# xmlyqing00/V-FloodNet

Hardware: AMD Instinct MI355X
Metric: segmented frames/sec at 480p (higher is better)
Workload: dtype f32

## Files before the change

v-floodnet_amd/_lib.py:

```python
import ctypes as C
import os
import re

import torch

_HERE = os.path.dirname(os.path.abspath(__file__))
LIB_PATH = os.environ.get('VFN_LIB_PATH') or os.path.join(_HERE, 'libvfn_hip.so')

_lib = None

c_fp = C.c_void_p

_SCALARS = {'int': C.c_int, 'float': C.c_float, 'double': C.c_double, 'long long': C.c_longlong}
_POINTEES = set(_SCALARS) | {'void', 'char', 'unsigned char', 'short', 'unsigned short', 'unsigned long long'}
_RENAMED = {'in': 'inp'}
_DECLARATOR = re.compile(r'(?:const\s+)?([A-Za-z_][\w ]*?)(?:\s*(\*)\s*|\s+)(\w+)\s*(?:\[([^\]]*)\])?')


def parse_header(text):
    defines, enums, structs, protos = {}, {}, {}, {}

    def fail(why, decl):
        raise RuntimeError(f'vfn_hip.h: {why}: {" ".join(decl.split())[:120]!r}')

    def number(expr, decl):
        try:
            if not re.fullmatch(r'[\w\s()+*-]+', expr):
                raise ValueError(expr)
            return int(eval(expr, {'__builtins__': {}}, {**defines, **enums}))
        except Exception:
            fail(f'cannot evaluate {expr.strip()!r}', decl)

    def declarator(item, decl, param):
        m = _DECLARATOR.fullmatch(item.strip())
        if not m:
            fail('declaration not understood', decl)
        base, star, name, bound = ' '.join(m.group(1).split()), m.group(2), m.group(3), m.group(4)
        if base not in _POINTEES and base not in structs:
            fail(f'unknown base type {base!r}', decl)
        if bound is not None and (star or param):
            fail('array of pointers or array parameter', decl)
        if star:
            if base == 'char':
                t = C.c_char_p
            elif base in structs and param and not name.endswith('_dev'):
                t = C.POINTER(structs[base])
            else:
                t = C.c_void_p
        elif base in _SCALARS:
            t = _SCALARS[base]
        elif base in structs and not param:
            t = structs[base]
        else:
            fail(f'{base!r} by value', decl)
        return _RENAMED.get(name, name), t if bound is None else t * number(bound, decl)

    text = re.sub(r'/\*.*?\*/', ' ', text, flags=re.S)
    text = re.sub(r'//[^\n]*', ' ', text)
    text = re.sub(r'^[ \t]*#[ \t]*ifdef[ \t]+__cplusplus\b.*?^[ \t]*#[ \t]*endif\b[^\n]*$', ' ', text, flags=re.S | re.M)
    code = []
    for line in text.split('\n'):
        if not line.lstrip().startswith('#'):
            code.append(line)
        elif not re.fullmatch(r'\s*#\s*(ifndef\s+\w+|define\s+\w+|endif)\s*', line):
            m = re.fullmatch(r'\s*#\s*define\s+(\w+)\b(?!\()(.+)', line)
            if not m:
                fail('directive not understood', line)
            defines[m.group(1)] = number(m.group(2), line)
    text = '\n'.join(code)

    decls, depth, start = [], 0, 0
    for pos, ch in enumerate(text):
        depth += (ch == '{') - (ch == '}')
        if depth < 0:
            fail('unbalanced declaration', text[start:pos + 1])
        if ch == ';' and depth == 0:
            decls.append(text[start:pos])
            start = pos + 1
    if text[start:].strip():
        fail('unbalanced declaration', text[start:])

    for decl in decls:
        m = re.fullmatch(r'\s*enum\s*\{(.*)\}\s*', decl, flags=re.S)
        if m:
            value = -1
            for item in m.group(1).split(','):
                name, _, expr = item.partition('=')
                value = number(expr, decl) if expr.strip() else value + 1
                enums[name.strip()] = value
            continue
        m = re.fullmatch(r'\s*typedef\s+struct\s*(\w*)\s*\{(.*)\}\s*(\w+)\s*', decl, flags=re.S)
        if m:
            if m.group(1) not in ('', m.group(3)):
                fail('struct tag and typedef name differ', decl)
            fields = []
            for member in m.group(2).split(';'):
                if member.strip():
                    first, *more = member.split(',')
                    head = _DECLARATOR.fullmatch(first.strip())
                    if more and (not head or head.group(2)):
                        fail('several declarators after a pointer', member)
                    fields.append(declarator(first, member, False))
                    fields += [declarator(f'{head.group(1)} {item}', member, False) for item in more]
            structs[m.group(3)] = type(m.group(3), (C.Structure,), {'_fields_': fields})
            continue
        m = re.fullmatch(r'\s*int\s+(vfn_\w+)\s*\((.*)\)\s*', decl, flags=re.S)
        if m:
            if m.group(1) in protos:
                fail('declared twice', decl)
            params = m.group(2).strip()
            protos[m.group(1)] = [] if params == 'void' else [declarator(p, decl, True)[1] for p in params.split(',')]
            continue
        fail('declaration not understood', decl)
    return defines, enums, structs, protos


with open(os.path.join(os.path.dirname(_HERE), 'include', 'vfn_hip.h')) as _f:
    DEFINES, ENUMS, STRUCTS, SIGNATURES = parse_header(_f.read())
ALL_SYMBOLS = sorted(SIGNATURES)
with open(os.path.join(os.path.dirname(_HERE), 'include', 'vfn_winograd6.h')) as _f:
    SIGNATURES_WINOGRAD6 = parse_header(_f.read())[3]
with open(os.path.join(os.path.dirname(_HERE), 'include', 'vfn_image_val.h')) as _f:
    DEFINES_IMAGE_VAL, _, _, SIGNATURES_IMAGE_VAL = parse_header(_f.read())
SEG_SCORES_CHUNK, SEG_SCORES_MAX_BLOCKS = DEFINES_IMAGE_VAL['VFN_SEG_SCORES_CHUNK'], DEFINES_IMAGE_VAL['VFN_SEG_SCORES_MAX_BLOCKS']
ABI_VERSION = DEFINES['VFN_ABI_VERSION']
TRAIN_AUG_MAX_T, TRAIN_AUG_MAX_SIDE, TRAIN_AUG_MAX_OUT, TRAIN_AUG_MAX_OBJ = (
    DEFINES['VFN_TRAIN_AUG_MAX_' + _k] for _k in ('T', 'SIDE', 'OUT', 'OBJ'))

ConvDesc = STRUCTS['vfn_conv_desc']
WgradDesc = STRUCTS['vfn_wgrad_desc']
RefreshFilter = STRUCTS['vfn_refresh_filter']
RefreshEpilogue = STRUCTS['vfn_refresh_epilogue']
GatherEntry = STRUCTS['vfn_gather_entry']
StemDesc = STRUCTS['vfn_stem_desc']
BankScanDesc = STRUCTS['vfn_bankscan_desc']
MemReadDesc = STRUCTS['vfn_memread_desc']
BankMatchDesc = STRUCTS['vfn_bankmatch_desc']
BankDesc = STRUCTS['vfn_bank_desc']
TrainAugFrame = STRUCTS['vfn_train_aug_frame']
TrainAugDesc = STRUCTS['vfn_train_aug_desc']

DESC_IDS = {ENUMS['VFN_DESC_' + _k]: _c for _k, _c in (
    ('CONV', ConvDesc), ('STEM', StemDesc), ('BANKSCAN', BankScanDesc), ('MEMREAD', MemReadDesc), ('BANK', BankDesc),
    ('WGRAD', WgradDesc), ('REFRESH_FILTER', RefreshFilter), ('REFRESH_EPILOGUE', RefreshEpilogue), ('GATHER', GatherEntry),
    ('BANKMATCH', BankMatchDesc), ('TRAIN_AUG', TrainAugDesc))}


def lib():
    global _lib
    if _lib is None:
        if not os.path.isfile(LIB_PATH):
            raise RuntimeError(
                f'{LIB_PATH} not found: build the HIP kernels first '
                '(python -c "import __graft_entry__ as g; g.build()" or make -C v-floodnet_amd/csrc)')
        L = C.CDLL(LIB_PATH)

        def declare(name, signatures=SIGNATURES, header='vfn_hip.h'):
            if not hasattr(L, name):
                raise RuntimeError(f'{LIB_PATH} lacks {name}, which include/{header} declares: rebuild it (make -C v-floodnet_amd/csrc)')
            fn = getattr(L, name)
            fn.argtypes, fn.restype = signatures[name], C.c_int
            return fn

        if declare('vfn_abi_version')() != ABI_VERSION:
            raise RuntimeError(f'{LIB_PATH} has ABI version {L.vfn_abi_version()}, this package expects {ABI_VERSION} '
                               '(descriptor layouts differ): rebuild it (make -C v-floodnet_amd/csrc)')
        declare('vfn_sizeof_desc')
        for which, cls in DESC_IDS.items():
            if L.vfn_sizeof_desc(which) != C.sizeof(cls):
                raise RuntimeError(f'{LIB_PATH}: sizeof({cls.__name__}) is {L.vfn_sizeof_desc(which)} in the library, '
                                   f'{C.sizeof(cls)} in this binding: rebuild it (make -C v-floodnet_amd/csrc)')
        for name in SIGNATURES:
            declare(name)
        for name in SIGNATURES_WINOGRAD6:
            declare(name, SIGNATURES_WINOGRAD6, 'vfn_winograd6.h')
        for name in SIGNATURES_IMAGE_VAL:
            declare(name, SIGNATURES_IMAGE_VAL, 'vfn_image_val.h')
        _lib = L
    return _lib


def check(status, what):
    if status != 0:
        raise RuntimeError(f'HIP kernel launcher {what} failed with status {status}')


def ptr(t):
    if t is None:
        return None
    return C.c_void_p(t.data_ptr())


_raw_stream = getattr(torch._C, '_cuda_getCurrentRawStream', None)


def stream():
    if _raw_stream is not None:
        return C.c_void_p(_raw_stream(torch.cuda.current_device()))
    return C.c_void_p(torch.cuda.current_stream().cuda_stream)


def require_gpu(t, what='tensor'):
    if not t.is_cuda:
        raise RuntimeError(f'{what} must live on the GPU: the V-FloodNet hot path has no CPU fallback')


PROBES = []


def independent_stream(device, beside=(), tries=12, priority=0):
    device = torch.device(device)
    cur = torch.cuda.current_stream(device)
    others = [cur] + [s_ for s_ in beside if s_ is not None]
    big, small = torch.zeros(16 * 1024 * 1024, device=device), torch.zeros(16, device=device)

    def overlaps(cand, ref):
        torch.cuda.synchronize(device)
        ref_end, cand_end = torch.cuda.Event(), torch.cuda.Event()
        with torch.cuda.stream(ref):
            for _ in range(64):
                big.add_(1.0)
            ref_end.record()
        with torch.cuda.stream(cand):
            small.add_(1.0)
            cand_end.record()
        cand_end.synchronize()
        ok = not ref_end.query()
        torch.cuda.synchronize(device)
        return ok

    cand = None
    for n_ in range(tries):
        cand = torch.cuda.Stream(device=device, priority=priority)
        if all(overlaps(cand, o_) for o_ in others):
            PROBES.append((True, n_ + 1))
            return cand
    PROBES.append((False, tries))
    import warnings
    warnings.warn('vfloodnet_amd: no stream with a hardware queue of its own found; side-stream work will run in order with the frame loop')
    return cand
```

v-floodnet_amd/csrc/conv_winograd.hip:

```cpp
#include "common.h"
#include "conv_internal.h"
#include "../../include/vfn_hip.h"
#include "../../include/vfn_winograd6.h"

namespace {

__device__ __forceinline__ void bt6(const f32x4 (&v)[6], f32x4 (&t)[6]) {
    t[0] = 4.f * v[0] - 5.f * v[2] + v[4];
    t[1] = -4.f * (v[1] + v[2]) + v[3] + v[4];
    t[2] = 4.f * (v[1] - v[2]) - v[3] + v[4];
    t[3] = -2.f * v[1] - v[2] + 2.f * v[3] + v[4];
    t[4] = 2.f * v[1] - v[2] - 2.f * v[3] + v[4];
    t[5] = 4.f * v[1] - 5.f * v[3] + v[5];
}

template <bool LPOUT = false>
__global__ __launch_bounds__(256)
void winograd_input_kernel(const float* __restrict__ x, int N, int H, int W, int C, int ld_x, int relu, float* __restrict__ V,
                           int rows_pad) {
    const int th = (H + 3) / 4, tw = (W + 3) / 4;
    const int c4n = C / 4;
    const long long total = (long long)N * th * tw * c4n;
    const __amdgpu_buffer_rsrc_t rx = __builtin_amdgcn_make_buffer_rsrc(const_cast<float*>(x), 0, (int)((size_t)N * H * W * ld_x * 4), 0x00020000);
    const float floor_ = relu ? 0.f : -INFINITY;
    for (long long i = vfn_xcd_block(blockIdx.x, gridDim.x) * (long long)blockDim.x + threadIdx.x; i < total; i += (long long)gridDim.x * blockDim.x) {
        const int c4 = (int)(i % c4n);
        const int tile = (int)(i / c4n);
        const int tx = tile % tw, ty = (tile / tw) % th, n = tile / (tw * th);
        f32x4 d[6][6];
#pragma unroll
        for (int a = 0; a < 6; ++a) {
            const int yy = 4 * ty - 1 + a;
#pragma unroll
            for (int b = 0; b < 6; ++b) {
                const int xx = 4 * tx - 1 + b;
                const bool ok = (unsigned)yy < (unsigned)H && (unsigned)xx < (unsigned)W;
                const int off = ok ? (((n * H + yy) * W + xx) * ld_x + c4 * 4) * 4 : 0x7ffffff0;
                d[a][b] = __builtin_bit_cast(f32x4, __builtin_amdgcn_raw_buffer_load_b128(rx, off, 0, 0));
            }
        }
#pragma unroll
        for (int a = 0; a < 6; ++a)
#pragma unroll
            for (int b = 0; b < 6; ++b)
#pragma unroll
                for (int e = 0; e < 4; ++e) d[a][b][e] = vfn_floor_nan(d[a][b][e], floor_);
#pragma unroll
        for (int b = 0; b < 6; ++b) {
            f32x4 v[6], t[6];
#pragma unroll
            for (int a = 0; a < 6; ++a) v[a] = d[a][b];
            bt6(v, t);
#pragma unroll
            for (int a = 0; a < 6; ++a) d[a][b] = t[a];
        }
#pragma unroll
        for (int a = 0; a < 6; ++a) {
            f32x4 t[6];
            bt6(d[a], t);
#pragma unroll
            for (int b = 0; b < 6; ++b) {
                if constexpr (LPOUT) {
                    const vfn_bf16x4 h = {(__bf16)t[b][0], (__bf16)t[b][1], (__bf16)t[b][2], (__bf16)t[b][3]};
                    *reinterpret_cast<vfn_bf16x4*>(reinterpret_cast<__bf16*>(V) + ((size_t)(a * 6 + b) * rows_pad + tile) * C + c4 * 4) = h;
                } else {
                    *reinterpret_cast<f32x4*>(V + ((size_t)(a * 6 + b) * rows_pad + tile) * C + c4 * 4) = t[b];
                }
            }
        }
    }
}

__device__ __forceinline__ void at6(const f32x4 (&m)[6], f32x4 (&y)[4]) {
    const f32x4 s12 = m[1] + m[2], d12 = m[1] - m[2], s34 = m[3] + m[4], d34 = m[3] - m[4];
    y[0] = m[0] + s12 + s34;
    y[1] = d12 + 2.f * d34;
    y[2] = s12 + 4.f * s34;
    y[3] = d12 + 8.f * d34 + m[5];
}

template <bool MASK>
__global__ __launch_bounds__(256)
void winograd_output_kernel(const float* __restrict__ Mb, int rows_pad, int N, int H, int W, int Cout,
                            const float* __restrict__ scale, const float* __restrict__ shift, const float* __restrict__ res, int res_ld,
                            int res_mod, int relu_out, float* __restrict__ out, int out_ld, const float* __restrict__ mask, int mask_ld,
                            int mask_after) {
    const int th = (H + 3) / 4, tw = (W + 3) / 4;
    const int c4n = Cout / 4;
    const long long total = (long long)N * th * tw * c4n;
    const int npix = N * H * W;
    const __amdgpu_buffer_rsrc_t ro = __builtin_amdgcn_make_buffer_rsrc(out, 0, (int)((size_t)npix * out_ld * 4), 0x00020000);
    const __amdgpu_buffer_rsrc_t rr = __builtin_amdgcn_make_buffer_rsrc(const_cast<float*>(res ? res : Mb), 0,
                                                                        res ? (int)((size_t)(res_mod > 0 ? res_mod : npix) * res_ld * 4) : 0, 0x00020000);
    const __amdgpu_buffer_rsrc_t rm = __builtin_amdgcn_make_buffer_rsrc(const_cast<float*>(MASK ? mask : Mb), 0,
                                                                        MASK ? (int)((size_t)npix * mask_ld * 4) : 0, 0x00020000);
    const float floor_ = relu_out ? 0.f : -INFINITY;
    for (long long i = vfn_xcd_block(blockIdx.x, gridDim.x) * (long long)blockDim.x + threadIdx.x; i < total; i += (long long)gridDim.x * blockDim.x) {
        const int c4 = (int)(i % c4n);
        const int tile = (int)(i / c4n);
        const int tx = tile % tw, ty = (tile / tw) % th, n = tile / (tw * th);
        f32x4 m[6][6];
#pragma unroll
        for (int a = 0; a < 6; ++a)
#pragma unroll
            for (int b = 0; b < 6; ++b) m[a][b] = *reinterpret_cast<const f32x4*>(Mb + ((size_t)(a * 6 + b) * rows_pad + tile) * Cout + c4 * 4);
        f32x4 sc = {1.f, 1.f, 1.f, 1.f}, sh = {0.f, 0.f, 0.f, 0.f};
        if (scale) sc = *reinterpret_cast<const f32x4*>(scale + c4 * 4);
        if (shift) sh = *reinterpret_cast<const f32x4*>(shift + c4 * 4);
        f32x4 t[6][4];
#pragma unroll
        for (int a = 0; a < 6; ++a) at6(m[a], t[a]);
        int rowi[4][4];
#pragma unroll
        for (int a = 0; a < 4; ++a)
#pragma unroll
            for (int b = 0; b < 4; ++b) {
                const int yy = 4 * ty + a, xx = 4 * tx + b;
                rowi[a][b] = (yy < H && xx < W) ? (n * H + yy) * W + xx : -1;
            }
        f32x4 rv[4][4], mk[MASK ? 4 : 1][MASK ? 4 : 1];
#pragma unroll
        for (int a = 0; a < 4; ++a)
#pragma unroll
            for (int b = 0; b < 4; ++b) {
                const int row = rowi[a][b];
                const int rrow = res_mod > 0 ? row % res_mod : row;
                rv[a][b] = __builtin_bit_cast(f32x4, __builtin_amdgcn_raw_buffer_load_b128(rr, row >= 0 ? (rrow * res_ld + c4 * 4) * 4 : 0x7ffffff0, 0, 0));
                if constexpr (MASK)
                    mk[a][b] = __builtin_bit_cast(f32x4, __builtin_amdgcn_raw_buffer_load_b128(rm, row >= 0 ? (row * mask_ld + c4 * 4) * 4 : 0x7ffffff0, 0, 0));
            }
#pragma unroll
        for (int b = 0; b < 4; ++b) {
            f32x4 col[6], y[4];
#pragma unroll
            for (int a = 0; a < 6; ++a) col[a] = t[a][b];
            at6(col, y);
#pragma unroll
            for (int a = 0; a < 4; ++a) {
                f32x4 v;
#pragma unroll
                for (int e = 0; e < 4; ++e) v[e] = y[a][e] * sc[e] + sh[e];
                if constexpr (MASK) {
                    if (!mask_after) {
#pragma unroll
                        for (int e = 0; e < 4; ++e) v[e] = mk[a][b][e] > 0.f ? v[e] : 0.f;
                    }
                }
                v += rv[a][b];
                if constexpr (MASK) {
                    if (mask_after) {
#pragma unroll
                        for (int e = 0; e < 4; ++e) v[e] = mk[a][b][e] > 0.f ? v[e] : 0.f;
                    }
                }
#pragma unroll
                for (int e = 0; e < 4; ++e) v[e] = vfn_floor_nan(v[e], floor_);
                const int row = rowi[a][b];
                __builtin_amdgcn_raw_buffer_store_b128(__builtin_bit_cast(__attribute__((ext_vector_type(4))) unsigned, v), ro,
                                                       row >= 0 ? (row * out_ld + c4 * 4) * 4 : 0x7ffffff0, 0, 0);
            }
        }
    }
}

typedef float f32x2 __attribute__((ext_vector_type(2)));
typedef unsigned u32x2 __attribute__((ext_vector_type(2)));

__device__ __forceinline__ void bt8(const f32x2 (&v)[8], f32x2 (&t)[8]) {
    const f32x2 e1 = v[2] + v[6] - 4.25f * v[4], o1 = v[1] + v[5] - 4.25f * v[3];
    const f32x2 e2 = v[6] + 0.25f * v[2] - 1.25f * v[4], o2 = 0.5f * v[1] - 2.5f * v[3] + 2.f * v[5];
    const f32x2 e3 = v[6] + 4.f * v[2] - 5.f * v[4], o3 = 2.f * v[1] - 2.5f * v[3] + 0.5f * v[5];
    t[0] = v[0] - v[6] + 5.25f * (v[4] - v[2]);
    t[1] = e1 + o1;
    t[2] = e1 - o1;
    t[3] = e2 + o2;
    t[4] = e2 - o2;
    t[5] = e3 + o3;
    t[6] = e3 - o3;
    t[7] = v[7] - v[1] + 5.25f * (v[3] - v[5]);
}

inline int winograd6_tiles(int N, int H, int W) { return N * ((H + 5) / 6) * ((W + 5) / 6); }

__global__ __launch_bounds__(256, 2)
void winograd6_input_kernel(const float* __restrict__ x, int N, int H, int W, int C, int ld_x, int relu, float* __restrict__ V,
                            int rows_pad) {
    const int th = (H + 5) / 6, tw = (W + 5) / 6, tiles = N * th * tw;
    const int c2n = C / 2;
    const long long total = (long long)rows_pad * c2n;
    const __amdgpu_buffer_rsrc_t rx = __builtin_amdgcn_make_buffer_rsrc(const_cast<float*>(x), 0, (int)((size_t)N * H * W * ld_x * 4), 0x00020000);
    const __amdgpu_buffer_rsrc_t rv = __builtin_amdgcn_make_buffer_rsrc(V, 0, (int)((size_t)64 * rows_pad * C * 4), 0x00020000);
    const int comp4 = rows_pad * C * 4;
    const float floor_ = relu ? 0.f : -INFINITY;
    const long long i = vfn_xcd_block(blockIdx.x, gridDim.x) * (long long)blockDim.x + threadIdx.x;
    if (i >= total) return;
    {
        const int c2 = (int)(i % c2n);
        const int tile = (int)(i / c2n);
        const int vo = (tile * C + c2 * 2) * 4;
        if (tile >= tiles) {
#pragma unroll
            for (int xi = 0; xi < 64; ++xi) __builtin_amdgcn_raw_buffer_store_b64(u32x2{0u, 0u}, rv, vo, xi * comp4, 0);
            return;
        }
        const int tx = tile % tw, ty = (tile / tw) % th, n = tile / (tw * th);
        const int y0 = 6 * ty - 1, x0 = 6 * tx - 1;
        const int base = (((n * H + y0) * W + x0) * ld_x + c2 * 2) * 4;
        f32x2 d[8][8];
#pragma unroll
        for (int a = 0; a < 8; ++a) {
#pragma unroll
            for (int b = 0; b < 8; ++b) {
                const bool ok = (unsigned)(y0 + a) < (unsigned)H && (unsigned)(x0 + b) < (unsigned)W;
                d[a][b] = __builtin_bit_cast(f32x2, __builtin_amdgcn_raw_buffer_load_b64(rx, ok ? base + (a * W + b) * ld_x * 4 : 0x7ffffff0, 0, 0));
            }
        }
#pragma unroll
        for (int a = 0; a < 8; ++a)
#pragma unroll
            for (int b = 0; b < 8; ++b)
#pragma unroll
                for (int e = 0; e < 2; ++e) d[a][b][e] = vfn_floor_nan(d[a][b][e], floor_);
#pragma unroll
        for (int b = 0; b < 8; ++b) {
            f32x2 v[8], t[8];
#pragma unroll
            for (int a = 0; a < 8; ++a) v[a] = d[a][b];
            bt8(v, t);
#pragma unroll
            for (int a = 0; a < 8; ++a) d[a][b] = t[a];
        }
#pragma unroll
        for (int a = 0; a < 8; ++a) {
            f32x2 t[8];
            bt8(d[a], t);
#pragma unroll
            for (int b = 0; b < 8; ++b) __builtin_amdgcn_raw_buffer_store_b64(__builtin_bit_cast(u32x2, t[b]), rv, vo, (a * 8 + b) * comp4, 0);
        }
    }
}

__device__ __forceinline__ void at8(const f32x2 (&m)[8], f32x2 (&y)[6]) {
    const f32x2 s12 = m[1] + m[2], d12 = m[1] - m[2], s34 = m[3] + m[4], d34 = m[3] - m[4], s56 = m[5] + m[6], d56 = m[5] - m[6];
    y[0] = m[0] + s12 + s34 + s56;
    y[1] = d12 + 2.f * d34 + 0.5f * d56;
    y[2] = s12 + 4.f * s34 + 0.25f * s56;
    y[3] = d12 + 8.f * d34 + 0.125f * d56;
    y[4] = s12 + 16.f * s34 + 0.0625f * s56;
    y[5] = d12 + 32.f * d34 + 0.03125f * d56 + m[7];
}

template <bool RES>
__global__ __launch_bounds__(256, RES ? 1 : 2)
void winograd6_output_kernel(const float* __restrict__ Mb, int rows_pad, int N, int H, int W, int Cout,
                             const float* __restrict__ scale, const float* __restrict__ shift, const float* __restrict__ res, int res_ld,
                             int res_mod, int relu_out, float* __restrict__ out, int out_ld) {
    const int th = (H + 5) / 6, tw = (W + 5) / 6;
    const int c2n = Cout / 2;
    const long long total = (long long)N * th * tw * c2n;
    const int npix = N * H * W;
    const __amdgpu_buffer_rsrc_t rm = __builtin_amdgcn_make_buffer_rsrc(const_cast<float*>(Mb), 0, (int)((size_t)64 * rows_pad * Cout * 4), 0x00020000);
    const __amdgpu_buffer_rsrc_t ro = __builtin_amdgcn_make_buffer_rsrc(out, 0, (int)((size_t)npix * out_ld * 4), 0x00020000);
    const __amdgpu_buffer_rsrc_t rr = __builtin_amdgcn_make_buffer_rsrc(const_cast<float*>(res ? res : Mb), 0,
                                                                        res ? (int)((size_t)(res_mod > 0 ? res_mod : npix) * res_ld * 4) : 0, 0x00020000);
    const float floor_ = relu_out ? 0.f : -INFINITY;
    const int comp4 = rows_pad * Cout * 4;
    const long long i = vfn_xcd_block(blockIdx.x, gridDim.x) * (long long)blockDim.x + threadIdx.x;
    if (i >= total) return;
    {
        int iw = (int)i;
        const int mo = ((iw / c2n) * Cout + (iw % c2n) * 2) * 4;
        f32x2 m[8][8];
#pragma unroll
        for (int a = 0; a < 8; ++a)
#pragma unroll
            for (int b = 0; b < 8; ++b) m[a][b] = __builtin_bit_cast(f32x2, __builtin_amdgcn_raw_buffer_load_b64(rm, mo, (a * 8 + b) * comp4, 0));
        f32x2 t[8][6];
#pragma unroll
        for (int a = 0; a < 8; ++a) at8(m[a], t[a]);
        __builtin_amdgcn_sched_barrier(0);
        asm volatile("" : "+v"(iw));
        const int c2 = iw % c2n, tile = iw / c2n;
        const int tx = tile % tw, ty = (tile / tw) % th, n = tile / (tw * th);
        f32x2 sc = {1.f, 1.f}, sh = {0.f, 0.f};
        if (scale) sc = *reinterpret_cast<const f32x2*>(scale + c2 * 2);
        if (shift) sh = *reinterpret_cast<const f32x2*>(shift + c2 * 2);
        const int y0 = 6 * ty, x0 = 6 * tx, row0 = (n * H + y0) * W + x0;
        const int rb = ((row0 - (res_mod > 0 ? (n * H * W) / res_mod * res_mod : 0)) * res_ld + c2 * 2) * 4;
        f32x2 rv[RES ? 6 : 1][RES ? 6 : 1];
        if constexpr (RES) {
#pragma unroll
            for (int a = 0; a < 6; ++a)
#pragma unroll
                for (int b = 0; b < 6; ++b) {
                    const bool ok = y0 + a < H && x0 + b < W;
                    rv[a][b] = __builtin_bit_cast(f32x2, __builtin_amdgcn_raw_buffer_load_b64(rr, ok ? rb + (a * W + b) * res_ld * 4 : 0x7ffffff0, 0, 0));
                }
        }
        const int oo = (row0 * out_ld + c2 * 2) * 4;
#pragma unroll
        for (int b = 0; b < 6; ++b) {
            f32x2 col[8], y[6];
#pragma unroll
            for (int a = 0; a < 8; ++a) col[a] = t[a][b];
            at8(col, y);
#pragma unroll
            for (int a = 0; a < 6; ++a) {
                f32x2 v;
#pragma unroll
                for (int e = 0; e < 2; ++e) v[e] = vfn_floor_nan(y[a][e] * sc[e] + sh[e] + (RES ? rv[a][b][e] : 0.f), floor_);
                const bool ok = y0 + a < H && x0 + b < W;
                __builtin_amdgcn_raw_buffer_store_b64(__builtin_bit_cast(u32x2, v), ro, ok ? oo + (a * W + b) * out_ld * 4 : 0x7ffffff0, 0, 0);
            }
        }
    }
}

__device__ __forceinline__ void a6(const f32x4 (&v)[4], f32x4 (&z)[6]) {
    const f32x4 e = v[0] + v[2], o = v[1] + v[3];
    const f32x4 e4 = v[0] + 4.f * v[2], o8 = 2.f * v[1] + 8.f * v[3];
    z[0] = v[0];
    z[1] = e + o;
    z[2] = e - o;
    z[3] = e4 + o8;
    z[4] = e4 - o8;
    z[5] = v[3];
}

__global__ __launch_bounds__(256)
void winograd_gy_kernel(const float* __restrict__ gy, int N, int H, int W, int C, int ld, float* __restrict__ Z, int rows_pad) {
    const int th = (H + 3) / 4, tw = (W + 3) / 4;
    const int c4n = C / 4;
    const long long total = (long long)N * th * tw * c4n;
    for (long long i = vfn_xcd_block(blockIdx.x, gridDim.x) * (long long)blockDim.x + threadIdx.x; i < total; i += (long long)gridDim.x * blockDim.x) {
        const int c4 = (int)(i % c4n);
        const int tile = (int)(i / c4n);
        const int tx = tile % tw, ty = (tile / tw) % th, n = tile / (tw * th);
        f32x4 t[6][4];
#pragma unroll
        for (int b = 0; b < 4; ++b) {
            f32x4 col[4], z[6];
            const int xx = 4 * tx + b;
#pragma unroll
            for (int a = 0; a < 4; ++a) {
                const int yy = 4 * ty + a;
                f32x4 v = {0.f, 0.f, 0.f, 0.f};
                if (yy < H && xx < W) v = *reinterpret_cast<const f32x4*>(gy + ((size_t)(n * H + yy) * W + xx) * ld + c4 * 4);
                col[a] = v;
            }
            a6(col, z);
#pragma unroll
            for (int a = 0; a < 6; ++a) t[a][b] = z[a];
        }
#pragma unroll
        for (int a = 0; a < 6; ++a) {
            f32x4 z[6];
            a6(t[a], z);
#pragma unroll
            for (int b = 0; b < 6; ++b)
                *reinterpret_cast<f32x4*>(Z + ((size_t)(a * 6 + b) * rows_pad + tile) * C + c4 * 4) = z[b];
        }
    }
}

__device__ __forceinline__ void gt3(const f32x4 (&u)[6], f32x4 (&w)[3]) {
    const f32x4 s12 = u[1] + u[2], d12 = u[2] - u[1], s34 = u[3] + u[4], d34 = u[3] - u[4];
    w[0] = 0.25f * u[0] - (1.f / 6.f) * s12 + (1.f / 24.f) * s34;
    w[1] = (1.f / 6.f) * d12 + (1.f / 12.f) * d34;
    w[2] = -(1.f / 6.f) * s12 + (1.f / 6.f) * s34 + u[5];
}

__global__ __launch_bounds__(256)
void winograd_dw_kernel(const float* __restrict__ dU, int Cout, int Cin, const float* __restrict__ rowscale, float* __restrict__ dw,
                        int accumulate) {
    const int c4n = Cin / 4;
    const long long total = (long long)Cout * c4n;
    const size_t bank = (size_t)Cout * Cin;
    for (long long i = vfn_xcd_block(blockIdx.x, gridDim.x) * (long long)blockDim.x + threadIdx.x; i < total; i += (long long)gridDim.x * blockDim.x) {
        const int c4 = (int)(i % c4n), co = (int)(i / c4n);
        f32x4 t[3][6];
#pragma unroll
        for (int j = 0; j < 6; ++j) {
            f32x4 u[6], w[3];
#pragma unroll
            for (int a = 0; a < 6; ++a) u[a] = *reinterpret_cast<const f32x4*>(dU + (size_t)(a * 6 + j) * bank + (size_t)co * Cin + c4 * 4);
            gt3(u, w);
#pragma unroll
            for (int a = 0; a < 3; ++a) t[a][j] = w[a];
        }
        const float sc = rowscale ? rowscale[co] : 1.f;
#pragma unroll
        for (int a = 0; a < 3; ++a) {
            f32x4 w[3];
            gt3(t[a], w);
#pragma unroll
            for (int b = 0; b < 3; ++b) {
                f32x4* o = reinterpret_cast<f32x4*>(dw + ((size_t)co * 9 + a * 3 + b) * Cin + c4 * 4);
                f32x4 v = w[b] * sc;
                if (accumulate) v += *o;
                *o = v;
            }
        }
    }
}


struct wino_gemm_args {
    const float* V;
    const float* U;
    float* Mb;
    int comps, rows_pad, C, Cout, cout_pad;
    int mtiles, ntiles;
    int a_ld, out_ld, res_ld, res_mod, relu_in, relu_out;
    const float* scale;
    const float* shift;
    const float* res;
};

template <int BM, int BN, int WM, int WN, int PD, bool CONV = false, bool LP = false>
__global__ __launch_bounds__(WM * WN * 64)
void wino_gemm_kernel(const wino_gemm_args p) {
    static_assert(!(CONV && LP), "the reduced-precision form is the transform-domain GEMM only");
    constexpr int BK = 32;
    constexpr int KT = LP ? 64 : 32;
    constexpr int ES = LP ? 2 : 4;
    constexpr int NT = WM * WN * 64;
    constexpr int TM = BM / WM / 32, TN = BN / WN / 32;
    constexpr int AC = BM * 8 / NT, BC = BN * 8 / NT, RSTEP = NT / 8;
    static_assert(AC >= 1 && BC >= 1, "tile too small for the thread count");
    extern __shared__ __attribute__((aligned(16))) char smem[];
    float* sA = reinterpret_cast<float*>(smem);
    float* sB = sA + 2 * BM * BK;

    const int tid = threadIdx.x, lane = tid & 63, wave = tid >> 6;
    const int wm = wave / WN, wn = wave % WN;
    const int li = lane & 31, lh = lane >> 5;

    const int per = p.mtiles * p.ntiles, total = p.comps * per;
    const int gx = (int)gridDim.x >> 3, xcd = (int)blockIdx.x & 7, loc = (int)blockIdx.x >> 3;
    const int q = total >> 3, r8 = total & 7;
    const int u_begin = xcd < r8 ? xcd * (q + 1) : r8 * (q + 1) + (xcd - r8) * q;
    const int u_end = u_begin + q + (xcd < r8 ? 1 : 0);
    const int first = u_begin + loc;
    const int n_units = first < u_end ? (u_end - first + gx - 1) / gx : 0;
    const int nk = p.C / KT;
    const int T = n_units * nk;
    if (T == 0) return;

    const int c16 = tid & 7, r0 = tid >> 3;
    const int a_ld = CONV ? p.a_ld : p.C;
    const __amdgpu_buffer_rsrc_t rsV = __builtin_amdgcn_make_buffer_rsrc(const_cast<float*>(p.V), 0, (int)((size_t)p.comps * p.rows_pad * a_ld * ES), 0x00020000);
    const __amdgpu_buffer_rsrc_t rsU = __builtin_amdgcn_make_buffer_rsrc(const_cast<float*>(p.U), 0, (int)((size_t)p.comps * p.cout_pad * p.C * ES), 0x00020000);
    int a_thr[AC], b_thr[BC];
#pragma unroll
    for (int j = 0; j < AC; ++j) a_thr[j] = (r0 + j * RSTEP) * a_ld * ES + c16 * 16;
#pragma unroll
    for (int j = 0; j < BC; ++j) b_thr[j] = (r0 + j * RSTEP) * p.C * ES + c16 * 16;

    int lu = 0, lkt = 0, la_base = 0, lb_base = 0;
    int n0_cur = 0;
    auto unit_bases = [&](int ui, int& a_base, int& b_base, size_t& o_base, int* n0 = nullptr) {
        const int u = first + ui * gx;
        const int xi = u / per, rem = u - xi * per;
        const int mt = rem / p.ntiles, nt = rem - mt * p.ntiles;
        a_base = (xi * p.rows_pad + mt * BM) * a_ld * ES;
        b_base = (xi * p.cout_pad + nt * BN) * p.C * ES;
        o_base = CONV ? (size_t)mt * BM : ((size_t)xi * p.rows_pad + mt * BM) * p.Cout + nt * BN;
        if (n0) *n0 = nt * BN;
    };
    size_t o_dummy;
    unit_bases(0, la_base, lb_base, o_dummy);
    f32x4 ra[PD][AC], rb[PD][BC];
    auto request = [&](int slot) {
        const int koff = lkt * 128;
#pragma unroll
        for (int j = 0; j < AC; ++j)
            ra[slot][j] = __builtin_bit_cast(f32x4, __builtin_amdgcn_raw_buffer_load_b128(rsV, a_thr[j], la_base + koff, 0));
#pragma unroll
        for (int j = 0; j < BC; ++j)
            rb[slot][j] = __builtin_bit_cast(f32x4, __builtin_amdgcn_raw_buffer_load_b128(rsU, b_thr[j], lb_base + koff, 0));
        if (++lkt == nk) {
            lkt = 0;
            if (++lu < n_units) unit_bases(lu, la_base, lb_base, o_dummy);
        }
    };
    const float relu_floor = (CONV && p.relu_in) ? 0.f : -INFINITY;
    auto stage = [&](int buf, int slot) {
        float* dA = sA + buf * BM * BK;
        float* dB = sB + buf * BN * BK;
#pragma unroll
        for (int j = 0; j < AC; ++j) {
            const int r = r0 + j * RSTEP;
            f32x4 v = ra[slot][j];
            if constexpr (CONV) {
#pragma unroll
                for (int e = 0; e < 4; ++e) v[e] = fmaxf(v[e], relu_floor);
            }
            *reinterpret_cast<f32x4*>(dA + r * BK + ((c16 ^ ((r >> 1) & 7)) << 2)) = v;
        }
#pragma unroll
        for (int j = 0; j < BC; ++j) {
            const int r = r0 + j * RSTEP;
            *reinterpret_cast<f32x4*>(dB + r * BK + ((c16 ^ ((r >> 1) & 7)) << 2)) = rb[slot][j];
        }
    };

    f32x16 acc[TM][TN];
#pragma unroll
    for (int i = 0; i < TM; ++i)
#pragma unroll
        for (int j = 0; j < TN; ++j)
#pragma unroll
            for (int r = 0; r < 16; ++r) acc[i][j][r] = 0.f;

    int cu = 0, ckt = 0, ca_dummy, cb_dummy;
    size_t o_base;
    unit_bases(0, ca_dummy, cb_dummy, o_base, &n0_cur);

#pragma unroll
    for (int d = 0; d < PD; ++d)
        if (d < T) request(d);
    stage(0, 0);
    __syncthreads();

    for (int t0 = 0; t0 < T; t0 += PD) {
#pragma unroll
        for (int uu = 0; uu < PD; ++uu) {
            const int t = t0 + uu;
            if (t >= T) break;
            const int buf = t & 1;
            const bool more = t + 1 < T;
            const bool more_req = t + PD < T;
            const float* cA = sA + buf * BM * BK + (wm * TM * 32) * BK;
            const float* cB = sB + buf * BN * BK + (wn * TN * 32) * BK;
            auto read_frags = [&](int kk, f32x4 (&a)[TM], f32x4 (&b)[TN]) {
                const int lc = 2 * kk + lh;
#pragma unroll
                for (int i = 0; i < TM; ++i) {
                    const int r = i * 32 + li;
                    a[i] = *reinterpret_cast<const f32x4*>(cA + r * BK + ((lc ^ ((r >> 1) & 7)) << 2));
                }
#pragma unroll
                for (int j = 0; j < TN; ++j) {
                    const int r = j * 32 + li;
                    b[j] = *reinterpret_cast<const f32x4*>(cB + r * BK + ((lc ^ ((r >> 1) & 7)) << 2));
                }
            };
            f32x4 fa[2][TM], fb[2][TN];
            read_frags(0, fa[0], fb[0]);
#pragma unroll
            for (int kk = 0; kk < 4; ++kk) {
                if (PD > 1 && kk == 0 && more) stage(buf ^ 1, (uu + 1) % PD);
                if (kk == 1 && more_req) request(uu);
                if (PD == 1 && kk == 3 && more) stage(buf ^ 1, 0);
                if (kk + 1 < 4) read_frags(kk + 1, fa[(kk + 1) & 1], fb[(kk + 1) & 1]);
                if constexpr (LP) {
                    typedef __attribute__((ext_vector_type(8))) __bf16 bf16x8_;
#pragma unroll
                    for (int i = 0; i < TM; ++i)
#pragma unroll
                        for (int j = 0; j < TN; ++j)
                            acc[i][j] = __builtin_amdgcn_mfma_f32_32x32x16_bf16(__builtin_bit_cast(bf16x8_, fa[kk & 1][i]), __builtin_bit_cast(bf16x8_, fb[kk & 1][j]),
                                                                                acc[i][j], 0, 0, 0);
                } else {
#pragma unroll
                for (int e = 0; e < 4; ++e)
#pragma unroll
                    for (int i = 0; i < TM; ++i)
#pragma unroll
                        for (int j = 0; j < TN; ++j)
                            acc[i][j] = __builtin_amdgcn_mfma_f32_32x32x2f32(fa[kk & 1][i][e], fb[kk & 1][j][e], acc[i][j], 0, 0, 0);
                }
            }
            if (++ckt == nk) {
                if constexpr (CONV) {
                    const int m0 = (int)o_base;
                    const int npix = p.rows_pad;
                    const __amdgpu_buffer_rsrc_t rso = __builtin_amdgcn_make_buffer_rsrc(p.Mb, 0, (int)((size_t)npix * p.out_ld * 4), 0x00020000);
                    const __amdgpu_buffer_rsrc_t rsr = __builtin_amdgcn_make_buffer_rsrc(const_cast<float*>(p.res ? p.res : p.V), 0,
                        p.res ? (int)((size_t)(p.res_mod > 0 ? p.res_mod : npix) * p.res_ld * 4) : 0, 0x00020000);
                    const float floor_ = p.relu_out ? 0.f : -INFINITY;
                    float rv[TM][TN][16];
#pragma unroll
                    for (int j = 0; j < TN; ++j) {
                        const int col = n0_cur + (wn * TN + j) * 32 + li;
#pragma unroll
                        for (int i = 0; i < TM; ++i)
#pragma unroll
                            for (int r = 0; r < 16; ++r) {
                                const int row = m0 + (wm * TM + i) * 32 + 4 * lh + (r & 3) + 8 * (r >> 2);
                                const int rrow = p.res_mod > 0 ? row % p.res_mod : row;
                                rv[i][j][r] = __builtin_bit_cast(float, __builtin_amdgcn_raw_buffer_load_b32(
                                    rsr, (row < npix && col < p.Cout) ? (rrow * p.res_ld + col) * 4 : 0x7ffffff0, 0, 0));
                            }
                    }
#pragma unroll
                    for (int j = 0; j < TN; ++j) {
                        const int col = n0_cur + (wn * TN + j) * 32 + li;
                        const bool cok = col < p.Cout;
                        const float sc = (p.scale && cok) ? p.scale[col] : 1.f;
                        const float sh = (p.shift && cok) ? p.shift[col] : 0.f;
#pragma unroll
                        for (int i = 0; i < TM; ++i)
#pragma unroll
                            for (int r = 0; r < 16; ++r) {
                                const int row = m0 + (wm * TM + i) * 32 + 4 * lh + (r & 3) + 8 * (r >> 2);
                                const float v = vfn_floor_nan(acc[i][j][r] * sc + sh + rv[i][j][r], floor_);
                                __builtin_amdgcn_raw_buffer_store_b32(__builtin_bit_cast(unsigned, v), rso,
                                                                      (row < npix && cok) ? (row * p.out_ld + col) * 4 : 0x7ffffff0, 0, 0);
                                acc[i][j][r] = 0.f;
                            }
                    }
                } else {
                float* o = p.Mb + o_base;
#pragma unroll
                for (int j = 0; j < TN; ++j) {
                    const int col = (wn * TN + j) * 32 + li;
#pragma unroll
                    for (int i = 0; i < TM; ++i) {
                        const int rbase = (wm * TM + i) * 32 + 4 * lh;
#pragma unroll
                        for (int r = 0; r < 16; ++r) {
                            if (n0_cur + col < p.Cout)
                                o[(size_t)(rbase + (r & 3) + 8 * (r >> 2)) * p.Cout + col] = acc[i][j][r];
                            acc[i][j][r] = 0.f;
                        }
                    }
                }
                }
                ckt = 0;
                if (++cu < n_units) unit_bases(cu, ca_dummy, cb_dummy, o_base, &n0_cur);
            }
            __syncthreads();
        }
    }
}

template <int BM, int BN, int WM, int WN, int PD, bool CONV, bool LP>
int launch_wino_gemm(const wino_gemm_args& a, int wgs, hipStream_t s) {
    constexpr size_t lds = 2 * (size_t)(BM + BN) * 32 * sizeof(float);
    static const bool lds_ready = vfn_allow_lds(&wino_gemm_kernel<BM, BN, WM, WN, PD, CONV, LP>, lds);
    (void)lds_ready;
    wino_gemm_args p = a;
    p.mtiles = (a.rows_pad + BM - 1) / BM;
    p.ntiles = (a.Cout + BN - 1) / BN;
    const int total = p.comps * p.mtiles * p.ntiles;
    int grid = wgs > 0 ? wgs : 512;
    if (grid > total) grid = total;
    grid = (grid + 7) / 8 * 8;
    hipLaunchKernelGGL((wino_gemm_kernel<BM, BN, WM, WN, PD, CONV, LP>), dim3(grid), dim3(WM * WN * 64), lds, s, p);
    return vfn_check_launch();
}

constexpr int kWinoTile[4][4] = {{128, 128, 4, 2}, {64, 128, 2, 4}, {128, 64, 4, 2}, {64, 64, 2, 2}};
constexpr int kWinoCfgs = 8;

template <bool CONV, bool LP>
int launch_wino_cfg(const wino_gemm_args& a, int cfg, int wgs, hipStream_t s) {
    return vfn_dispatch<kWinoCfgs>(cfg, [&](auto id) -> int {
        constexpr int c = decltype(id)::value;
        constexpr const int* t = kWinoTile[c & 3];
        return launch_wino_gemm<t[0], t[1], t[2], t[3], 1 + (c >> 2), CONV, LP>(a, wgs, s);
    });
}

inline bool tensors_fit_32bit(int N, int H, int W, int ld, int res_ld, int mask_ld, int res_mod) {
    const long long px = (long long)N * H * W;
    return px * ld * 4 < 0x7fffff00LL && (res_mod > 0 ? (long long)res_mod : px) * res_ld * 4 < 0x7fffff00LL && px * mask_ld * 4 < 0x7fffff00LL;
}

inline int grid_of(long long total) {
    long long b = (total + 255) / 256;
    return (int)(b < 16384 ? (b ? b : 1) : 16384);
}

}

extern "C" int vfn_winograd_tiles(int N, int H, int W) { return N * ((H + 3) / 4) * ((W + 3) / 4); }

extern "C" int vfn_winograd_input_f32(const float* x, int N, int H, int W, int C, int ld_x, int relu, float* V, int rows_pad, void* stream) {
    if (!x || !V || N < 1 || H < 1 || W < 1 || C < 4 || C % 4 || ld_x < C || ld_x % 4 || rows_pad < vfn_winograd_tiles(N, H, W)) return VFN_ERR_ARG;
    const long long total = (long long)vfn_winograd_tiles(N, H, W) * (C / 4);
    if (!tensors_fit_32bit(N, H, W, ld_x, 0, 0, 0)) return VFN_ERR_ARG;
    hipLaunchKernelGGL(winograd_input_kernel<false>, dim3(grid_of(total)), dim3(256), 0, (hipStream_t)stream, x, N, H, W, C, ld_x, relu, V, rows_pad);
    return vfn_check_launch();
}

extern "C" int vfn_winograd_output_f32(const float* Mb, int rows_pad, int N, int H, int W, int Cout, const float* scale, const float* shift,
                                       const float* res, int res_ld, int res_mod, int relu_out, float* out, int out_ld, void* stream) {
    if (!Mb || !out || N < 1 || H < 1 || W < 1 || Cout < 4 || Cout % 4 || out_ld < Cout || out_ld % 4 || (res && res_ld % 4) ||
        rows_pad < vfn_winograd_tiles(N, H, W)) return VFN_ERR_ARG;
    const long long total = (long long)vfn_winograd_tiles(N, H, W) * (Cout / 4);
    if (!tensors_fit_32bit(N, H, W, out_ld, res ? res_ld : 0, 0, res_mod)) return VFN_ERR_ARG;
    hipLaunchKernelGGL(winograd_output_kernel<false>, dim3(grid_of(total)), dim3(256), 0, (hipStream_t)stream, Mb, rows_pad, N, H, W, Cout, scale, shift,
                       res, res_ld, res_mod, relu_out, out, out_ld, (const float*)nullptr, 0, 0);
    return vfn_check_launch();
}

extern "C" int vfn_winograd6_input_f32(const float* x, int N, int H, int W, int C, int ld_x, int relu, float* V, int rows_pad, void* stream) {
    if (!x || !V || N < 1 || H < 1 || W < 1 || C < 4 || C % 4 || ld_x < C || ld_x % 4 || rows_pad < winograd6_tiles(N, H, W)) return VFN_ERR_ARG;
    if (!tensors_fit_32bit(N, H, W, ld_x, 0, 0, 0) || (long long)64 * rows_pad * C * 4 >= 0x7fffff00LL) return VFN_ERR_ARG;
    hipLaunchKernelGGL(winograd6_input_kernel, dim3(((long long)rows_pad * (C / 2) + 255) / 256), dim3(256), 0, (hipStream_t)stream, x, N, H, W, C, ld_x, relu,
                       V, rows_pad);
    return vfn_check_launch();
}

extern "C" int vfn_winograd6_output_f32(const float* Mb, int rows_pad, int N, int H, int W, int Cout, const float* scale, const float* shift,
                                        const float* res, int res_ld, int res_mod, int relu_out, float* out, int out_ld, void* stream) {
    if (!Mb || !out || N < 1 || H < 1 || W < 1 || Cout < 4 || Cout % 4 || out_ld < Cout || out_ld % 4 || (res && res_ld % 4) ||
        rows_pad < winograd6_tiles(N, H, W) || res_mod < 0 || (res && res_mod % (H * W))) return VFN_ERR_ARG;
    if (!tensors_fit_32bit(N, H, W, out_ld, res ? res_ld : 0, 0, res_mod) || (long long)64 * rows_pad * Cout * 4 >= 0x7fffff00LL) return VFN_ERR_ARG;
    const dim3 grid(((long long)winograd6_tiles(N, H, W) * (Cout / 2) + 255) / 256);
    if (res)
        hipLaunchKernelGGL(winograd6_output_kernel<true>, grid, dim3(256), 0, (hipStream_t)stream, Mb, rows_pad, N, H, W, Cout, scale, shift, res, res_ld,
                           res_mod, relu_out, out, out_ld);
    else
        hipLaunchKernelGGL(winograd6_output_kernel<false>, grid, dim3(256), 0, (hipStream_t)stream, Mb, rows_pad, N, H, W, Cout, scale, shift, res, res_ld,
                           res_mod, relu_out, out, out_ld);
    return vfn_check_launch();
}

extern "C" int vfn_winograd_output_masked_f32(const float* Mb, int rows_pad, int N, int H, int W, int Cout, const float* res, int res_ld,
                                              const float* mask, int mask_ld, int mask_after, float* out, int out_ld, void* stream) {
    if (!Mb || !out || N < 1 || H < 1 || W < 1 || Cout < 4 || Cout % 4 || out_ld < Cout || out_ld % 4 || (res && res_ld % 4) ||
        (mask && mask_ld % 4) || rows_pad < vfn_winograd_tiles(N, H, W)) return VFN_ERR_ARG;
    const long long total = (long long)vfn_winograd_tiles(N, H, W) * (Cout / 4);
    if (!tensors_fit_32bit(N, H, W, out_ld, res ? res_ld : 0, mask ? mask_ld : 0, 0)) return VFN_ERR_ARG;
    if (mask)
        hipLaunchKernelGGL(winograd_output_kernel<true>, dim3(grid_of(total)), dim3(256), 0, (hipStream_t)stream, Mb, rows_pad, N, H, W, Cout,
                           (const float*)nullptr, (const float*)nullptr, res, res_ld, 0, 0, out, out_ld, mask, mask_ld, mask_after);
    else
        hipLaunchKernelGGL(winograd_output_kernel<false>, dim3(grid_of(total)), dim3(256), 0, (hipStream_t)stream, Mb, rows_pad, N, H, W, Cout,
                           (const float*)nullptr, (const float*)nullptr, res, res_ld, 0, 0, out, out_ld, (const float*)nullptr, 0, 0);
    return vfn_check_launch();
}

extern "C" int vfn_winograd_gy_f32(const float* gy, int N, int H, int W, int C, int ld, float* Z, int rows_pad, void* stream) {
    if (!gy || !Z || N < 1 || H < 1 || W < 1 || C < 4 || C % 4 || ld < C || ld % 4 || rows_pad < vfn_winograd_tiles(N, H, W)) return VFN_ERR_ARG;
    const long long total = (long long)vfn_winograd_tiles(N, H, W) * (C / 4);
    hipLaunchKernelGGL(winograd_gy_kernel, dim3(grid_of(total)), dim3(256), 0, (hipStream_t)stream, gy, N, H, W, C, ld, Z, rows_pad);
    return vfn_check_launch();
}

extern "C" int vfn_winograd_dw_f32(const float* dU, int Cout, int Cin, const float* rowscale, float* dw, int accumulate, void* stream) {
    if (!dU || !dw || Cout < 1 || Cin < 4 || Cin % 4) return VFN_ERR_ARG;
    hipLaunchKernelGGL(winograd_dw_kernel, dim3(grid_of((long long)Cout * (Cin / 4))), dim3(256), 0, (hipStream_t)stream, dU, Cout, Cin, rowscale,
                       dw, accumulate);
    return vfn_check_launch();
}

extern "C" int vfn_winograd_gemm_f32(const float* V, const float* U, float* Mb, int comps, int rows_pad, int C, int Cout, int cout_pad, int cfg,
                                     int wgs, void* stream) {
    if (!V || !U || !Mb || comps < 1 || rows_pad < 1 || C < 32 || C % 32 || Cout < 1 || cout_pad < Cout || cfg < 0 || cfg >= kWinoCfgs) return VFN_ERR_ARG;
    const int bm = kWinoTile[cfg & 3][0], bn = kWinoTile[cfg & 3][1];
    if (rows_pad % bm || cout_pad < (Cout + bn - 1) / bn * bn) return VFN_ERR_ARG;
    if ((long long)comps * rows_pad * C * 4 >= 0x7fffff00LL || (long long)comps * cout_pad * C * 4 >= 0x7fffff00LL) return VFN_ERR_ARG;
    wino_gemm_args a{V, U, Mb, comps, rows_pad, C, Cout, cout_pad, 0, 0, 0, 0, 0, 0, 0, 0, nullptr, nullptr, nullptr};
    return launch_wino_cfg<false, false>(a, cfg, wgs, (hipStream_t)stream);
}

extern "C" int vfn_conv1x1_persistent_f32(const vfn_conv_desc* d, int cfg, int wgs, void* stream) {
    if (!d || !d->in || !d->w || !d->out || cfg < 0 || cfg >= kWinoCfgs) return VFN_ERR_ARG;
    if (d->KH != 1 || d->KW != 1 || d->stride != 1 || d->pad != 0 || d->mask || d->in_lp || d->out_lp || d->w_packed || d->ksplit > 1 ||
        d->w_batch_rows || d->Cin % 32 || d->in_ld % 4 || d->M < 1 || d->M != d->N * d->H * d->W) return VFN_ERR_ARG;
    const int bn = kWinoTile[cfg & 3][1];
    if (d->cout_pad < (d->Cout + bn - 1) / bn * bn) return VFN_ERR_ARG;
    const long long lim = 0x7fffff00LL;
    if ((long long)d->M * d->in_ld * 4 >= lim || (long long)d->M * d->out_ld * 4 >= lim || (long long)d->cout_pad * d->Cin * 4 >= lim ||
        (d->res && (long long)(d->res_mod > 0 ? d->res_mod : d->M) * d->res_ld * 4 >= lim)) return VFN_ERR_ARG;
    wino_gemm_args a{d->in, d->w, d->out, 1, d->M, d->Cin, d->Cout, d->cout_pad, 0, 0,
                     d->in_ld, d->out_ld, d->res ? d->res_ld : 0, d->res_mod, d->relu_in, d->relu_out, d->scale, d->shift, d->res};
    return launch_wino_cfg<true, false>(a, cfg, wgs, (hipStream_t)stream);
}

extern "C" int vfn_winograd_input_bf16(const float* x, int N, int H, int W, int C, int ld_x, int relu, void* V, int rows_pad, void* stream) {
    if (!x || !V || N < 1 || H < 1 || W < 1 || C < 4 || C % 4 || ld_x < C || ld_x % 4 || rows_pad < vfn_winograd_tiles(N, H, W)) return VFN_ERR_ARG;
    const long long total = (long long)vfn_winograd_tiles(N, H, W) * (C / 4);
    if (!tensors_fit_32bit(N, H, W, ld_x, 0, 0, 0)) return VFN_ERR_ARG;
    hipLaunchKernelGGL(winograd_input_kernel<true>, dim3(grid_of(total)), dim3(256), 0, (hipStream_t)stream, x, N, H, W, C, ld_x, relu,
                       reinterpret_cast<float*>(V), rows_pad);
    return vfn_check_launch();
}

extern "C" int vfn_winograd_gemm_bf16(const void* V, const void* U, float* Mb, int comps, int rows_pad, int C, int Cout, int cout_pad, int cfg,
                                      int wgs, void* stream) {
    if (!V || !U || !Mb || comps < 1 || rows_pad < 1 || C < 64 || C % 64 || Cout < 1 || cout_pad < Cout || cfg < 0 || cfg >= kWinoCfgs) return VFN_ERR_ARG;
    const int bm = kWinoTile[cfg & 3][0], bn = kWinoTile[cfg & 3][1];
    if (rows_pad % bm || cout_pad < (Cout + bn - 1) / bn * bn) return VFN_ERR_ARG;
    if ((long long)comps * rows_pad * C * 2 >= 0x7fffff00LL || (long long)comps * cout_pad * C * 2 >= 0x7fffff00LL) return VFN_ERR_ARG;
    wino_gemm_args a{reinterpret_cast<const float*>(V), reinterpret_cast<const float*>(U), Mb, comps, rows_pad, C, Cout, cout_pad, 0, 0, 0, 0, 0, 0, 0, 0,
                     nullptr, nullptr, nullptr};
    return launch_wino_cfg<false, true>(a, cfg, wgs, (hipStream_t)stream);
}
```

v-floodnet_amd/engine.py:

```python
import math
import os

import torch

from . import _lib, ops, weights as W
from ._lib import ptr, stream, check, MemReadDesc, BankScanDesc
from .feature_bank import pick_nsplit, pick_scan_slices, MAX_SPLIT, MAX_SPLIT_SCAN, QT_SCAN, DK, DV

_CFG_EFF = {(128, 128): 1.00, (128, 64): 0.95, (64, 128): 0.95, (64, 64): 0.86, (32, 64): 0.74,
            (64, 32): 0.74, (128, 32): 0.80, (256, 128): 0.97}
_CFG_TILES = None
_TUNED = {}
_TUNED_PATH = __import__('os').path.join(__import__('os').path.dirname(__import__('os').path.abspath(__file__)),
                                         'tuned_gfx950.json')
_TUNED_BF16 = {}
_TUNED_BF16_PATH = _TUNED_PATH.replace('tuned_gfx950.json', 'tuned_gfx950_bf16.json')
_TUNED_BF16X3 = {}
_TUNED_BF16X3_PATH = _TUNED_PATH.replace('tuned_gfx950.json', 'tuned_gfx950_bf16x3.json')
_TABLES = (_TUNED, _TUNED_BF16, _TUNED_BF16X3)
_TABLE_PATHS = (_TUNED_PATH, _TUNED_BF16_PATH, _TUNED_BF16X3_PATH)
_TUNED_WINO6 = {}
_TUNED_WINO6_PATH = _TUNED_PATH.replace('tuned_gfx950.json', 'tuned_gfx950_wino6.json')


def is_wino6_desc(d):
    return d.w_batch_rows > 0 and d.M == 64 * d.w_batch_rows


def table_of(d, mode):
    return _TUNED_WINO6 if mode == 0 and is_wino6_desc(d) else _TABLES[mode]


def _load_tuned():
    import json
    import os
    if os.environ.get('VFN_IGNORE_TUNED') == '1':
        return
    for path, table in zip(_TABLE_PATHS + (_TUNED_WINO6_PATH,), _TABLES + (_TUNED_WINO6,)):
        alt = os.environ.get('VFN_TUNED_DIR')
        if alt and os.path.isfile(os.path.join(alt, os.path.basename(path))):
            path = os.path.join(alt, os.path.basename(path))
        if os.path.isfile(path):
            for k, v in json.load(open(path)).items():
                t = (int(v[0]), int(v[1]), int(v[2]) if len(v) > 2 else 0)
                table[tuple(int(x) for x in k.split(','))] = t + tuple(int(x) for x in v[3:6]) if len(v) >= 6 else t


def save_tuned(path=None, mode=0):
    import json
    table = _TUNED_WINO6 if mode == 'wino6' else _TABLES[mode]
    with open(path or (_TUNED_WINO6_PATH if mode == 'wino6' else _TABLE_PATHS[mode]), 'w') as f:
        json.dump({','.join(str(x) for x in k): list(v) for k, v in sorted(table.items())}, f, indent=0)


_load_tuned()


def pad_divide_by(h, w, d=16):
    new_h = h + d - h % d if h % d > 0 else h
    new_w = w + d - w % d if w % d > 0 else w
    lh = int((new_h - h) / 2)
    uh = int(new_h - h) - lh
    lw = int((new_w - w) / 2)
    uw = int(new_w - w) - lw
    return (lw, uw, lh, uh), new_h, new_w


WS_FLOATS = 16 * 1024 * 1024
_WINOGRAD_TRAIN = os.environ.get('VFN_WINOGRAD_TRAIN', '1') == '1'
_BATCH_MEMREAD = os.environ.get('VFN_TRAIN_BATCH_MEMREAD', '1') == '1'
MAX_GROUP = 16
_TRAIN_SLOTS = int(os.environ.get('VFN_TRAIN_SLOTS', 2))
_WINOGRAD = os.environ.get('VFN_WINOGRAD', '1')
_WINOGRAD_F6 = os.environ.get('VFN_WINOGRAD_F6', '1')
_WINOGRAD_LP = os.environ.get('VFN_WINOGRAD_LP', '1') == '1'
_WINOGRAD_MIN_M = int(os.environ.get('VFN_WINOGRAD_MIN_M', 10000))
_WINO_TABLE = {}
_WINO_TABLE_BF16 = {}
_WINO_PATH = os.path.join(os.path.dirname(os.path.abspath(__file__)), 'wino_gfx950.json')
if os.environ.get('VFN_IGNORE_TUNED') != '1':
    for _path, _tab in ((_WINO_PATH, _WINO_TABLE), (_WINO_PATH.replace('.json', '_bf16.json'), _WINO_TABLE_BF16)):
        if os.path.isfile(_path):
            _tab.update({tuple(int(x) for x in k.split(',')): int(v) for k, v in __import__('json').load(open(_path)).items()})
_INLAUNCH_SPLITK = __import__('os').environ.get('VFN_INLAUNCH_SPLITK', '1') == '1'


def _tiles():
    global _CFG_TILES
    if _CFG_TILES is None:
        _CFG_TILES = ops.conv_cfg_tiles()
    return _CFG_TILES


def apply_choice(desc, choice, ws, counters=None):
    cfg, ks, split_from = choice[:3]
    if ks > 1 and (desc.out_ld % 4 or (desc.res and desc.res_ld % 4)):
        ks, split_from = 1, 0
    if cfg >= ops.PCONV_CFG0 and not ops.pconv_eligible(desc, 0):
        fb = tuple(choice[3:6]) if len(choice) >= 6 else choose_cfg(desc.M, desc.Cout, desc.KH * desc.KW * desc.Cin, 0, use_table=False)
        return apply_choice(desc, fb, ws, counters)
    if cfg >= ops.WINO_GEMM_CFG0:
        ops.set_splitk(desc, 1, None)
        return cfg
    if ops.conv_cfg_kind(cfg) == 2:
        if counters is None or ws is None or ws.numel() < ops.SK_WS_FLOATS:
            ws, counters = ops.streamk_scratch(ws.device if ws is not None else torch.device('cuda', torch.cuda.current_device()))
        ops.set_streamk(desc, ws, counters)
        return cfg
    if ks > 1:
        bm, bn = _tiles()[cfg]
        n_tiles = (desc.Cout + bn - 1) // bn
        rows = desc.M - (split_from // n_tiles) * bm
        if desc.Cout % bn or not _INLAUNCH_SPLITK or ops.conv_cfg_kind(cfg) != 0 or desc.w_packed or desc.in_lp or desc.out_lp:
            counters = None
        ops.set_splitk(desc, ks, ws, split_from, rows, counters)
    else:
        ops.set_splitk(desc, 1, None)
    return cfg


def _scores_buffer(p, fb):
    if os.environ.get('VFN_STORE_SCORES', '1') == '0':
        return None
    per_obj = ((fb._cap + 63) // 64) * ((p.HW + 127) // 128) * 8192
    if fb.obj_n * per_obj * 4 > float(os.environ.get('VFN_SCORES_MAX_GB', 48)) * 2 ** 30:
        return None
    key = (fb.obj_n, per_obj)
    if getattr(p, '_scores_key', None) != key:
        p._scores = torch.empty(fb.obj_n, per_obj, device=p.dec_in.device)
        p._scores_key = key
    return p._scores


def choose_cfg(M, cout, K, mode=0, use_table=True):
    global _CFG_TILES
    key = (M, cout, K)
    table = _TABLES[mode]
    if use_table and key in table:
        return table[key]
    _tiles()
    nk = K // (64 if mode == 1 else 32)
    best, best_cost = 0, None
    for c, (bm, bn) in enumerate(_CFG_TILES[:8]):
        if bn > 32 and cout <= 32:
            continue
        if bn >= 128 and cout < 128:
            continue
        blocks = ((M + bm - 1) // bm) * ((cout + bn - 1) // bn)
        rounds = (blocks + 255) // 256
        cost = rounds * bm * bn / _CFG_EFF[(bm, bn)]
        if best_cost is None or cost < best_cost:
            best, best_cost = c, cost
    c = 2 if cout >= 128 else 3
    bm, bn = _CFG_TILES[c]
    blocks = ((M + bm - 1) // bm) * ((cout + bn - 1) // bn)
    if blocks < 200 and nk >= 16 and cout % 4 == 0 and cout >= 64:
        ks = max(1, min(16, (448 + blocks - 1) // blocks, nk // 4))
        while ks > 1 and (((nk + ks - 1) // ks) * (ks - 1) >= nk or ks * M * cout > WS_FLOATS):
            ks -= 1
        return (c, ks, 0)
    return (best, 1, 0)


def tune_desc(d, bf, ws, cnt, iters=3, cfg_filter=None, allow_split=True):
    tiles = ops.conv_cfg_tiles()
    key = (d.M, d.Cout, d.KH * d.KW * d.Cin)

    def timeit(c):
        ops.conv2d_launch(d, c, bf)
        torch.cuda.synchronize()
        best_ms = None
        for _ in range(3):
            e0, e1 = torch.cuda.Event(enable_timing=True), torch.cuda.Event(enable_timing=True)
            e0.record()
            for _ in range(iters):
                ops.conv2d_launch(d, c, bf)
            e1.record()
            torch.cuda.synchronize()
            ms = e0.elapsed_time(e1)
            best_ms = ms if best_ms is None else min(best_ms, ms)
        return best_ms

    best, best_t = None, None
    if d.w_batch_rows > 0 and bf == 1:
        for c in ops.wino_gemm_cfg_options(d.w_batch_rows, d.Cout):
            if cfg_filter is not None and not cfg_filter(key, c):
                continue
            t = timeit(c)
            if best_t is None or t < best_t:
                best, best_t = (c, 1, 0), t
        return best
    if d.w_batch_rows > 0 and bf == 0 and d.M // d.w_batch_rows * d.w_batch_rows == d.M:
        for c in ops.wino_gemm_cfg_options(d.w_batch_rows, d.Cout):
            if cfg_filter is not None and not cfg_filter(key, c):
                continue
            apply_choice(d, (c, 1, 0), ws, cnt)
            try:
                t = timeit(c)
            except RuntimeError:
                continue
            if best_t is None or t < best_t:
                best, best_t = (c, 1, 0), t
    if ops.pconv_eligible(d, bf) and os.environ.get('VFN_PCONV', '1') == '1':
        for c in ops.pconv_cfg_options(d.Cout):
            if cfg_filter is not None and not cfg_filter(key, c):
                continue
            apply_choice(d, (c, 1, 0), ws, cnt)
            try:
                t = timeit(c)
            except RuntimeError:
                continue
            if best_t is None or t < best_t:
                best, best_t = (c, 1, 0), t
    for c, (bm, bn) in enumerate(tiles):
        if c not in ops.conv_cfgs(bf):
            continue
        if cfg_filter is not None and not cfg_filter(key, c):
            continue
        if d.cout_pad < ((d.Cout + bn - 1) // bn) * bn or (d.w_batch_rows > 0 and d.w_batch_rows % bm):
            continue
        if (bn > 64 and d.Cout <= 32) or (bn > 128 and d.Cout < 256):
            continue
        blocks = ((d.M + bm - 1) // bm) * ((d.Cout + bn - 1) // bn)
        options = [(c, 1, 0)]
        wk = ops.conv_cfg_wk(c)
        kind = ops.conv_cfg_kind(c)
        if kind == 2:
            if blocks > ops.SK_MAX_TILES:
                continue
        elif not allow_split:
            pass
        elif kind == 1 and wk > 1:
            if blocks < 256:
                options += [(c, k_, 0) for k_ in ops.valid_splits(d, 8, bf)[1:] if k_ * d.M * d.Cout <= WS_FLOATS]
        elif wk > 1 or ops.conv_cfg_tpb(c) > 1:
            if blocks > 1024 or d.KH * d.KW * d.Cin // (64 if bf == 1 else 32) < 2 * wk:
                continue
        elif blocks < 256:
            options += [(c, k_, 0) for k_ in ops.valid_splits(d, 16, bf)[1:] if k_ * d.M * d.Cout <= WS_FLOATS]
        else:
            options += [(c, k_, full) for (full, k_, rows) in ops.tail_split_options(d, bm, bn, 8, bf)
                        if k_ * rows * d.Cout <= WS_FLOATS and k_ in (2, 3, 4, 5, 6, 8)]
        for opt in options:
            apply_choice(d, opt, ws, cnt)
            t = timeit(c)
            if best_t is None or t < best_t:
                best, best_t = opt, t
    return best


class ConvLayer:

    def __init__(self, conv, bn=None, device=None, cin_range=None, with_bias=True, reg=None):
        w = conv.weight.detach().float()
        if cin_range is not None:
            w = w[:, cin_range[0]:cin_range[1]].contiguous()
        self.cout, self.cin, self.k, _ = w.shape
        self.stride = conv.stride[0]
        self.pad = conv.padding[0]
        self.w = ops.pad_rows(W.pack_conv_weight(w)).to(device)
        sc, sh = W.conv_epilogue(conv, bn)
        if not with_bias:
            sh = torch.zeros_like(sh)
        self.scale = sc.to(device).contiguous()
        self.shift = sh.to(device).contiguous()
        self._w_lp = {}
        self._wino_src = None
        if reg is not None and isinstance(conv, torch.nn.Module):
            from .refresh import FORWARD
            self._wino_src = [(reg, conv.weight, cin_range[0] if cin_range is not None else 0, 0)]
            reg.add_filter(conv.weight, self.w, FORWARD, cin=self.cin, cin_off=cin_range[0] if cin_range is not None else 0)
            if bn is not None:
                reg.add_epilogue(self.scale, self.shift if with_bias else None, bn=bn, eps=W.BN_EPS)
            elif conv.bias is not None and with_bias:
                reg.add_epilogue(None, self.shift, bias=conv.bias)

    def refresh_derived(self):
        for mode, t in self._w_lp.items():
            if mode == 'wino':
                if self._wino_src is not None:
                    continue
                w = self.w[:self.cout].view(self.cout, 3, 3, self.cin).permute(0, 3, 1, 2)
                t.copy_(ops.pack_winograd_weight(w).to(t.device))
            elif mode == 'wino6':
                if self._wino_src is not None:
                    continue
                w = self.w[:self.cout].view(self.cout, 3, 3, self.cin).permute(0, 3, 1, 2)
                t.copy_(ops.pack_winograd6_weight(w).to(t.device))
            elif mode == 'wino_bf16':
                w = self.w[:self.cout].view(self.cout, 3, 3, self.cin).permute(0, 3, 1, 2)
                t.copy_(ops.pack_winograd_weight_bf16(w).to(t.device))
            else:
                new = ops.pack_weights_lp(self.w, mode)
                t.copy_(new)

    def w_lp(self, mode):
        if mode not in self._w_lp:
            self._w_lp[mode] = ops.pack_weights_lp(self.w, mode)
        return self._w_lp[mode]

    def w_wino(self):
        if 'wino' not in self._w_lp:
            assert self.k == 3
            w = self.w[:self.cout].view(self.cout, 3, 3, self.cin).permute(0, 3, 1, 2)
            self._w_lp['wino'] = ops.pack_winograd_weight(w).to(self.w.device)
            if self._wino_src is not None:
                from .refresh import WINO
                for reg, weight, cin_off, row0 in self._wino_src:
                    reg.add_filter(weight, self._w_lp['wino'], WINO, cin=self.cin, cin_off=cin_off, dst_ld=self.cin, dst_row0=row0,
                                   cout_ld=self._w_lp['wino'].shape[0] // 36)
        return self._w_lp['wino']

    def w_wino6(self):
        if 'wino6' not in self._w_lp:
            assert self.k == 3
            w = self.w[:self.cout].view(self.cout, 3, 3, self.cin).permute(0, 3, 1, 2)
            self._w_lp['wino6'] = ops.pack_winograd6_weight(w).to(self.w.device)
            if self._wino_src is not None:
                from .refresh import WINO6
                for reg, weight, cin_off, row0 in self._wino_src:
                    reg.add_filter(weight, self._w_lp['wino6'], WINO6, cin=self.cin, cin_off=cin_off, dst_ld=self.cin, dst_row0=row0,
                                   cout_ld=self._w_lp['wino6'].shape[0] // 64)
        return self._w_lp['wino6']

    def w_wino_bf16(self):
        if 'wino_bf16' not in self._w_lp:
            assert self.k == 3
            w = self.w[:self.cout].view(self.cout, 3, 3, self.cin).permute(0, 3, 1, 2)
            self._w_lp['wino_bf16'] = ops.pack_winograd_weight_bf16(w).to(self.w.device)
        return self._w_lp['wino_bf16']


class Pred2Layer:
    TAPS = 20

    def __init__(self, conv, device, reg=None):
        w = conv.weight.detach().float().cpu()
        assert w.shape[0] == 2 and w.shape[2:] == (3, 3)
        self.cin = w.shape[1]
        w18 = torch.zeros(self.TAPS, self.cin)
        for dy in range(3):
            for dx in range(3):
                for o in range(2):
                    w18[(dy * 3 + dx) * 2 + o] = w[o, :, dy, dx]
        self.cout, self.k, self.stride, self.pad = self.TAPS, 1, 1, 0
        self.w = ops.pad_rows(w18.contiguous()).to(device)
        self.scale = torch.ones(self.TAPS, device=device)
        self.shift = torch.zeros(self.TAPS, device=device)
        self.bias = conv.bias.detach().float().to(device).contiguous().clone()
        self._w_lp = {}
        self._wino_src = None
        if reg is not None:
            from .refresh import TAPS
            reg.add_filter(conv.weight, self.w, TAPS)
            reg.add_epilogue(None, self.bias, bias=conv.bias)

    refresh_derived = ConvLayer.refresh_derived

    def w_lp(self, mode):
        if mode not in self._w_lp:
            self._w_lp[mode] = ops.pack_weights_lp(self.w, mode)
        return self._w_lp[mode]


class Launch:
    __slots__ = ('fn', 'args', 'name', 'flops')

    def __init__(self, fn, args, name, flops=0.0):
        self.fn, self.args, self.name, self.flops = fn, args, name, flops

    def __call__(self):
        self.fn(*self.args)


_GRAPHS = os.environ.get('VFN_GRAPHS', '1') == '1'


class GraphCache:

    def __init__(self):
        self.graphs = {}
        self.runs = {}
        self.captures = 0

    def invalidate(self):
        self.graphs.clear()
        self.runs.clear()

    def run(self, lst, lo=0, hi=None, eager=False):
        hi = len(lst) if hi is None else hi
        if hi <= lo:
            return
        key = (id(lst), lo, hi)
        g = None if (eager or not _GRAPHS) else self.graphs.get(key)
        if g is not None:
            g.replay()
            return
        n = self.runs.get(key, 0)
        if eager or not _GRAPHS or n < 2 or hi - lo < 4:
            for l in lst[lo:hi]:
                l()
            if not eager:
                self.runs[key] = n + 1
            return
        g = torch.cuda.CUDAGraph()
        cur = torch.cuda.current_stream()
        cap = torch.cuda.Stream(device=cur.device)
        cap.wait_stream(cur)
        try:
            with torch.cuda.graph(g, stream=cap, capture_error_mode='thread_local'):
                for l in lst[lo:hi]:
                    l()
        except Exception:
            import warnings
            warnings.warn('vfloodnet_amd: HIP graph capture of a launch list failed; running it eagerly')
            self.runs[key] = -10 ** 9
            if torch.cuda.is_current_stream_capturing():
                raise RuntimeError('vfloodnet_amd: the stream is still capturing after a failed HIP graph capture')
            cur.wait_stream(cap)
            for l in lst[lo:hi]:
                l()
            return
        cur.wait_stream(cap)
        self.graphs[key] = g
        self.captures += 1
        g.replay()

    def warm(self, lst, lo=0, hi=None):
        hi = len(lst) if hi is None else hi
        if not _GRAPHS or hi - lo < 4:
            return
        key = (id(lst), lo, hi)
        while key not in self.graphs and self.runs.get(key, 0) >= 0:
            self.run(lst, lo, hi)


class FramePlan:

    def __init__(self, eng, H0, W0, obj_n, keep_acts=False):
        self.eng = eng
        self.graphs = GraphCache()
        self.keep_acts = keep_acts
        self.acts_m = {}
        self.H0, self.W0, self.obj_n = H0, W0, obj_n
        self.pad, self.Hp, self.Wp = pad_divide_by(H0, W0)
        dev = eng.device
        self.h2, self.w2 = self.Hp // 2, self.Wp // 2
        self.h4, self.w4 = self.Hp // 4, self.Wp // 4
        self.h8, self.w8 = self.Hp // 8, self.Wp // 8
        self.h16, self.w16 = self.Hp // 16, self.Wp // 16
        self.HW = self.h16 * self.w16
        f = lambda *s: torch.empty(*s, device=dev, dtype=torch.float32)
        K = obj_n
        self.frame_in = f(3, H0, W0)
        self.mask_in = f(K, H0, W0)
        self.qsets = [QuerySet(self), QuerySet(self)]
        self._qbatch = {}
        self.m = self._trunk_buffers(K)
        self.kv_m = f(K, self.HW, DK + DV)
        self.ml = f(K, self.HW, 2)
        self.ml_part = f(K, MAX_SPLIT_SCAN, self.HW, 2)
        self.work = torch.zeros(4, dtype=torch.int32, device=dev)
        self.o_part = f(K, MAX_SPLIT, self.HW, DV)
        self.dec_in = f(K, self.h16, self.w16, DV)
        self.d16 = [f(K, self.h16, self.w16, 256) for _ in range(3)]
        self.d8 = [f(K, self.h8, self.w8, 256) for _ in range(3)]
        self.d4 = [f(K, self.h4, self.w4, 256) for _ in range(3)]
        self.pp = f(K, self.h4, self.w4, 2)
        self.z4 = f(K, self.h4, self.w4, Pred2Layer.TAPS)
        self.z2 = f(K, self.h2, self.w2, Pred2Layer.TAPS)
        self.p_up = f(K, self.h2, self.w2, 2)
        self.rough = f(K, self.h2, self.w2)
        self.unc = f(self.h2, self.w2)
        fused_ok = K <= 4
        self.hs = None if fused_ok else f(K, self.h2, self.w2, 64)
        self.hr = None if fused_ok else f(K, self.h2, self.w2)
        self.hm = None if fused_ok else f(K, self.h2, self.w2)
        self.lm = f(K, self.h2, self.w2, 64)
        self.conf = f(K, self.h2, self.w2)
        self.l2 = [f(K, self.h2, self.w2, 32) for _ in range(3)]
        self.qq = f(K, self.h2, self.w2, 2)
        self.score = f(1, K, H0, W0)
        self._twins = {}
        self._lp_state = {}
        self.ws = f(WS_FLOATS)
        self.ws_q = f(WS_FLOATS)
        self.cnt = torch.zeros(ops.SK_MAX_TILES, dtype=torch.int32, device=dev)
        self.cnt_q = torch.zeros(ops.SK_MAX_TILES, dtype=torch.int32, device=dev)
        self._ws_cur, self._cnt_cur = self.ws, self.cnt
        self._wino = {}

        self.mem = []
        self._build()

    @property
    def seg_pre(self):
        return self.qsets[0].pre[1]

    @property
    def seg_post(self):
        return self.qsets[0].post[0]

    @property
    def kv_q(self):
        return self.qsets[0].kv_q[0:1]

    def all_lists(self):
        out = [self.mem]
        for qs in self.qsets:
            out += [qs.pre[1], qs.pre[2], qs.post[0], qs.post[1]]
        for qs in self._qbatch.values():
            out += [qs.pre[qs.nq]]
            if qs._dec_batch is not None:
                out += [qs._dec_batch.post]
        return out

    def batch_set(self, n):
        qs = self._qbatch.get(n)
        if qs is None:
            qs = self._qbatch[n] = QuerySet(self, nq=n)
            qs.build()
        return qs

    def _trunk_buffers(self, N):
        dev = self.eng.device
        f = lambda *s: torch.empty(*s, device=dev, dtype=torch.float32)
        b = {}
        b['r1'] = f(N, self.h2, self.w2, 64)
        b['x4'] = f(N, self.h4, self.w4, 64)
        for name, (h, w, planes) in {'res2': (self.h4, self.w4, 64), 'res3': (self.h8, self.w8, 128),
                                     'res4': (self.h16, self.w16, 256)}.items():
            hin, win = (h * 2, w * 2) if name != 'res2' else (h, w)
            b[name] = dict(t1a=f(N, hin, win, planes), t1=f(N, h, w, planes), t2=f(N, h, w, planes),
                           ds=f(N, h, w, planes * 4), o=[f(N, h, w, planes * 4) for _ in range(2)],
                           out=f(N, h, w, planes * 4))
        return b

    def _lp_args(self, out):
        if not self.eng.any_x3 or out.shape[-1] % 32:
            return ()
        self._lp_state[(out.data_ptr(), tuple(out.shape))] = True
        return (self.lp_twin(out), True)

    def lp_twin(self, t):
        st = t.untyped_storage()
        key = st.data_ptr()
        if key not in self._twins:
            self._twins[key] = torch.empty(st.nbytes() // 4, dtype=torch.float32, device=t.device)
        return torch.as_strided(self._twins[key], t.size(), t.stride(), t.storage_offset())

    def has_lp(self, t, relu):
        return self._lp_state.get((t.data_ptr(), tuple(t.shape))) == bool(relu)

    def _conv(self, lst, layer, x, out, N, H, Wd, res=None, relu_in=False, relu_out=False, name='conv',
              in_ld=None, out_ld=None, res_mod=0, lp_out=None, f32_out=True):
        bf = self.eng.layer_mode(name)
        lp = bf == 2
        if self.eng.mixed:
            f32_out = True
        if ((bf == 0 or (bf == 1 and _WINOGRAD_LP and not self.keep_acts and layer.cin % 64 == 0)) and in_ld is None and
                (_WINOGRAD_TRAIN or not self.keep_acts) and x.shape[-1] == layer.cin and self.eng.use_winograd(layer, N * H * Wd, bf)):
            tile = 6 if (bf == 0 and not self.keep_acts and res_mod % (H * Wd) == 0 and
                         self.eng.winograd_tile(layer, N * H * Wd) == 6) else 4
            return self._conv_winograd(lst, layer, x, out, N, H, Wd, res, relu_in, relu_out, name, out_ld, res_mod, bf, tile)
        d = ops.make_conv_desc(x, layer.w, layer.cout, layer.k, layer.k, layer.stride, layer.pad, out,
                               layer.scale, layer.shift, res, relu_in, relu_out,
                               cin=layer.cin, in_ld=in_ld if in_ld is not None else x.shape[-1],
                               out_ld=out_ld, N=N, H=H, W=Wd)
        d.res_mod = int(res_mod)
        if lp and in_ld is None and layer.cin % 32 == 0 and self.has_lp(x, relu_in):
            d.inp, d.in_lp, d.relu_in = ptr(self.lp_twin(x)), 1, 0
        if lp and lp_out and layer.cout % 32 == 0 and d.out_ld % 32 == 0:
            d.out_lp, d.out_lp_relu = ptr(self.lp_twin(out)), int(lp_out == 'relu')
            self._lp_state[(out.data_ptr(), tuple(out.shape))] = (lp_out == 'relu')
            if not f32_out:
                d.out = None
        else:
            self._lp_state.pop((out.data_ptr(), tuple(out.shape)), None)
        K = layer.k * layer.k * layer.cin
        if bf == 1 and layer.cin % 64:
            bf = 2
        if bf:
            ops.use_packed_weights(d, layer.w_lp(bf))
        choice = choose_cfg(d.M, layer.cout, K, bf)
        if choice[1] > 1 and (d.out_ld % 4 or (res is not None and d.res_ld % 4)):
            choice = (choice[0], 1, 0)
        cfg = apply_choice(d, choice, self._ws_cur, self._cnt_cur)
        lst.append(Launch(ops.conv2d_launch, (d, cfg, bf), f'{name}[{d.M}x{layer.cout}x{K}]', 2.0 * d.M * layer.cout * K))
        return out

    def _conv_winograd(self, lst, layer, x, out, N, H, Wd, res, relu_in, relu_out, name, out_ld, res_mod, bf=0, tile=4):
        comps = 64 if tile == 6 else 36
        rows = ops.winograd6_rows(N, H, Wd) if tile == 6 else ops.winograd_rows(N, H, Wd)
        key = id(self._ws_cur)
        need_v, need_m = comps * rows * layer.cin, comps * rows * layer.cout
        V, Mb = self._wino.get(key, (None, None))
        if V is None or V.numel() < need_v or Mb.numel() < need_m:
            dev = self.eng.device
            V = torch.zeros(max(need_v, V.numel() if V is not None else 0), device=dev)
            Mb = torch.empty(max(need_m, Mb.numel() if Mb is not None else 0), device=dev)
            self._wino[key] = (V, Mb)
        Mb = Mb[:need_m].view(comps * rows, layer.cout)
        if bf == 1:
            V = V.view(torch.bfloat16)[:need_v].view(36 * rows, layer.cin)
            U = layer.w_wino_bf16()
        else:
            V = V[:need_v].view(comps * rows, layer.cin)
            U = layer.w_wino6() if tile == 6 else layer.w_wino()
        lst.append(Launch(ops.winograd_input, (x, V, rows, relu_in, N, H, Wd, layer.cin, x.shape[-1], tile), name + '.wino_in'))
        dg = ops.make_winograd_gemm_desc(V, U, Mb, rows, layer.cin, layer.cout, comps)
        if bf:
            choice = _TABLES[bf].get((dg.M, layer.cout, layer.cin))
            if choice is None or choice[0] < ops.WINO_GEMM_CFG0:
                tc = 5 if rows % 64 == 0 and layer.cout >= 128 and rows >= 1024 else 3
                choice = (ops.wino_gemm_cfg(tc, 512), 1, 0)
        elif tile == 6:
            choice = _TUNED_WINO6.get((dg.M, layer.cout, layer.cin))
            if choice is None or choice[0] not in ops.wino_gemm_cfg_options(rows, layer.cout):
                choice = (ops.wino_gemm_cfg(5 if layer.cout >= 128 else 7, 768), 1, 0)
        else:
            choice = choose_cfg(dg.M, layer.cout, layer.cin, 0)
        cfg = apply_choice(dg, choice, self._ws_cur, self._cnt_cur)
        lst.append(Launch(ops.conv2d_launch, (dg, cfg, bf), f'{name}.wino_gemm[{dg.M}x{layer.cout}x{layer.cin}]', 2.0 * dg.M * layer.cout * layer.cin))
        self._lp_state.pop((out.data_ptr(), tuple(out.shape)), None)
        lst.append(Launch(ops.winograd_output, (Mb, rows, out, N, H, Wd, layer.cout, layer.scale, layer.shift, res,
                                                res.shape[-1] if res is not None else 0, res_mod, relu_out,
                                                out_ld if out_ld is not None else out.shape[-1], tile), name + '.wino_out'))
        return out

    def _trunk(self, lst, enc, bufs, N, prefix, acts=None):
        x = bufs['x4']
        lst.append(Launch(ops.maxpool3x3s2, (bufs['r1'], x), prefix + '.maxpool'))
        H, Wd = self.h4, self.w4
        for lname in ('res2', 'res3', 'res4'):
            blocks = enc[lname]
            lb = bufs[lname]
            for bi, blk in enumerate(blocks):
                s = blk['conv2'].stride
                Ho, Wo = H // s, Wd // s
                t1 = lb['t1a'] if (s == 2) else lb['t1']
                t2, ds_buf = lb['t2'], lb['ds']
                if self.keep_acts:
                    t1, t2 = torch.empty_like(t1), torch.empty_like(lb['t2'])
                    ds_buf = torch.empty_like(lb['ds'])
                nm = f'{prefix}.{lname}.{bi}'
                self._conv(lst, blk['conv1'], x, t1, N, H, Wd, relu_out=True, name=nm + '.conv1', lp_out='plain', f32_out=False)
                self._conv(lst, blk['conv2'], t1, t2, N, H, Wd, relu_out=True, name=nm + '.conv2', lp_out='plain',
                           f32_out=False)
                if 'down' in blk:
                    self._conv(lst, blk['down'], x, ds_buf, N, H, Wd, name=nm + '.down')
                    idn = ds_buf
                else:
                    idn = x
                out = lb['out'] if bi == len(blocks) - 1 else lb['o'][bi % 2]
                if self.keep_acts and bi != len(blocks) - 1:
                    out = torch.empty_like(out)
                self._conv(lst, blk['conv3'], t2, out, N, Ho, Wo, res=idn, relu_out=True, name=nm + '.conv3',
                           lp_out='plain')
                if self.keep_acts and acts is not None:
                    acts[(lname, bi)] = dict(x=x, t1=t1, t2=t2, ds=ds_buf if 'down' in blk else None, out=out, stride=s, H=H, W=Wd)
                x = out
                H, Wd = Ho, Wo
        return x

    def _resblock(self, lst, rb, x, t, out, N, H, Wd, name):
        self._conv(lst, rb['conv1'], x, t, N, H, Wd, relu_in=True, name=name + '.conv1', lp_out='relu', f32_out=False)
        self._conv(lst, rb['conv2'], t, out, N, H, Wd, res=x, relu_in=True, name=name + '.conv2')
        return out

    def _build(self):
        e = self.eng
        K = self.obj_n
        for qs in self.qsets:
            qs.build()
        self._ws_cur, self._cnt_cur = self.ws, self.cnt
        self.stem_m = ops.make_stem_desc(self.frame_in, self.mask_in, e.stem_m_w, e.stem_m_scale, e.stem_m_shift,
                                         self.m['r1'], e.mean, e.std, K, self.H0, self.W0, self.pad, self.Hp, self.Wp)
        self.mem.append(Launch(ops.stem_launch, (self.stem_m,), 'encoder_m.stem',
                               2.0 * K * self.h2 * self.w2 * 64 * 245))
        r4m = self._trunk(self.mem, e.enc_m, self.m, K, 'encoder_m', acts=self.acts_m)
        self._conv(self.mem, e.keyval, r4m, self.kv_m, K, self.h16, self.w16, name='keyval')

    def conv_flops(self, which):
        return sum(l.flops for l in getattr(self, which))


class QuerySet:

    def __init__(self, plan, nq=2):
        self.plan = plan
        self.nq = nq
        p = plan
        f = lambda *s_: torch.empty(*s_, device=p.eng.device, dtype=torch.float32)
        self.frames = f(nq, 3, p.H0, p.W0)
        self.q = p._trunk_buffers(nq)
        self.kv_q = f(nq, p.HW, DK + DV)
        self.fm_q = f(nq, p.h16, p.w16, 256)
        self.s8 = [f(nq, p.h8, p.w8, 256) for _ in range(3)]
        self.s4 = [f(nq, p.h4, p.w4, 256) for _ in range(3)]
        self.lq = f(nq, p.h2, p.w2, 32)
        self.sizes = sorted({1, nq})
        self.pre = {n: [] for n in self.sizes}
        self.acts = {n: {} for n in self.sizes}
        self.post = [[] for _ in range(nq)]
        self.split = {n: 0 for n in self.sizes}
        self.keys = [None] * nq
        self.held = [None] * nq
        self.consumed = [True] * nq
        self.stage = 0
        self.n = 0
        self.done = None
        self._dec_batch = None

    def dec_batch(self):
        if self._dec_batch is None:
            self._dec_batch = DecoderBatch(self.plan, self)
        return self._dec_batch

    @staticmethod
    def _sl(t, n):
        return t[0:n]

    def build(self):
        p, e = self.plan, self.plan.eng
        K = p.obj_n
        D = e.dec
        for n in self.sizes:
            P = self.pre[n]
            sl = lambda t: t[0:n]
            q = {k: (sl(v) if torch.is_tensor(v) else {kk: ([sl(x) for x in vv] if isinstance(vv, list) else sl(vv)) for kk, vv in v.items()})
                 for k, v in self.q.items()}
            p._ws_cur, p._cnt_cur = p.ws_q, p.cnt_q
            for i in range(n):
                d = ops.make_stem_desc(self.frames[i], None, e.stem_q_w, e.stem_q_scale, e.stem_q_shift,
                                       self.q['r1'][i:i + 1], e.mean, e.std, 1, p.H0, p.W0, p.pad, p.Hp, p.Wp)
                P.append(Launch(ops.stem_launch, (d,), 'encoder_q.stem', 2.0 * p.h2 * p.w2 * 64 * 147))
            r4 = p._trunk(P, e.enc_q, q, n, 'encoder_q', acts=self.acts[n])
            p._conv(P, e.keyval, r4, sl(self.kv_q), n, p.h16, p.w16, name='keyval')
            kvq_val = sl(self.kv_q)[:, :, DK:]
            p._conv(P, D['convFM_q'], kvq_val, sl(self.fm_q), n, p.h16, p.w16, name='decoder.convFM.q', in_ld=DK + DV)
            s8, s4 = [sl(t) for t in self.s8], [sl(t) for t in self.s4]
            p._conv(P, D['RF3']['convFS'], q['res3']['out'], s8[0], n, p.h8, p.w8, name='decoder.RF3.convFS', lp_out='relu')
            p._resblock(P, D['RF3']['ResFS'], s8[0], s8[1], s8[2], n, p.h8, p.w8, 'decoder.RF3.ResFS')
            p._conv(P, D['RF2']['convFS'], q['res2']['out'], s4[0], n, p.h4, p.w4, name='decoder.RF2.convFS', lp_out='relu')
            p._resblock(P, D['RF2']['ResFS'], s4[0], s4[1], s4[2], n, p.h4, p.w4, 'decoder.RF2.ResFS')
            p._conv(P, D['local_convFM_r1'], q['r1'], sl(self.lq), n, p.h2, p.w2, name='decoder.local_convFM.r1')
            est = [l.flops / 100e12 + 6e-6 for l in P]
            half, acc = 0.5 * sum(est), 0.0
            for i, t_ in enumerate(est):
                acc += t_
                if acc >= half:
                    self.split[n] = i + 1
                    break
        p._ws_cur, p._cnt_cur = p.ws, p.cnt
        d16, d8, d4 = p.d16, p.d8, p.d4
        for slot in range(self.nq):
            L = self.post[slot]
            o = lambda t: t[slot:slot + 1]
            p._conv(L, D['convFM_m'], p.dec_in, d16[0], K, p.h16, p.w16, res=o(self.fm_q), res_mod=p.HW,
                    name='decoder.convFM.mem', lp_out='relu')
            p._resblock(L, D['ResMM'], d16[0], d16[1], d16[2], K, p.h16, p.w16, 'decoder.ResMM')
            L.append(Launch(ops.upsample2x_add, (o(self.s8[2]), d16[2], d8[0], True) + p._lp_args(d8[0]), 'decoder.RF3.up_add'))
            p._resblock(L, D['RF3']['ResMM'], d8[0], d8[1], d8[2], K, p.h8, p.w8, 'decoder.RF3.ResMM')
            L.append(Launch(ops.upsample2x_add, (o(self.s4[2]), d8[2], d4[0], True) + p._lp_args(d4[0]), 'decoder.RF2.up_add'))
            p._resblock(L, D['RF2']['ResMM'], d4[0], d4[1], d4[2], K, p.h4, p.w4, 'decoder.RF2.ResMM')
            p._conv(L, D['pred2'], d4[2], p.z4, K, p.h4, p.w4, relu_in=True, name='decoder.pred2.taps')
            L.append(Launch(ops.pred2_gather, (p.z4, D['pred2'].bias, p.pp), 'decoder.pred2.gather'))
            L.append(Launch(ops.rough_uncertainty, (p.pp, p.p_up, p.rough, p.unc), 'decoder.rough_unc'))
            L.append(Launch(ops.local_stats, (self.q['r1'][slot], p.rough, p.hs, p.hr, p.hm, p.lm, p.conf),
                            'decoder.local_stats'))
            l2 = p.l2
            p._conv(L, D['local_convFM_loc'], p.lm, l2[0], K, p.h2, p.w2, res=o(self.lq),
                    res_mod=p.h2 * p.w2, name='decoder.local_convFM.local', lp_out='relu')
            p._resblock(L, D['local_ResMM'], l2[0], l2[1], l2[2], K, p.h2, p.w2, 'decoder.local_ResMM')
            p._conv(L, D['local_pred2'], l2[2], p.z2, K, p.h2, p.w2, relu_in=True, name='decoder.local_pred2.taps')
            L.append(Launch(ops.pred2_gather, (p.z2, D['local_pred2'].bias, p.qq), 'decoder.local_pred2.gather'))
            L.append(Launch(ops.final_logits, (p.p_up, p.unc, p.conf, p.qq, p.score, p.pad, p.H0, p.W0), 'decoder.final_logits'))


class DecoderBatch:

    def __init__(self, plan, qs):
        self.plan, self.qs, self.G = plan, qs, qs.nq
        p, G, K = plan, qs.nq, plan.obj_n
        N = G * K
        self.N = N
        f = lambda *s_: torch.empty(*s_, device=p.eng.device, dtype=torch.float32)
        self.dec_in = f(N, p.h16, p.w16, DV)
        self.d16 = [f(N, p.h16, p.w16, 256) for _ in range(3)]
        self.d8 = [f(N, p.h8, p.w8, 256) for _ in range(3)]
        self.d4 = [f(N, p.h4, p.w4, 256) for _ in range(3)]
        self.pp = f(N, p.h4, p.w4, 2)
        self.z4 = f(N, p.h4, p.w4, Pred2Layer.TAPS)
        self.z2 = f(N, p.h2, p.w2, Pred2Layer.TAPS)
        self.p_up = f(N, p.h2, p.w2, 2)
        self.rough = f(N, p.h2, p.w2)
        self.unc = f(G, p.h2, p.w2)
        self.lm = f(N, p.h2, p.w2, 64)
        self.conf = f(N, p.h2, p.w2)
        self.l2 = [f(N, p.h2, p.w2, 32) for _ in range(3)]
        self.qq = f(N, p.h2, p.w2, 2)
        self.score = f(G, K, p.H0, p.W0)
        self._mr = None
        self.post = []
        self._build()

    @property
    def mr(self):
        if self._mr is None:
            import types
            p, G, K = self.plan, self.G, self.plan.obj_n
            f = lambda *s_: torch.empty(*s_, device=p.eng.device, dtype=torch.float32)
            HWb = G * p.HW
            self._mr = types.SimpleNamespace(HW=HWb, ml=f(K, HWb, 2), ml_part=f(K, MAX_SPLIT_SCAN, HWb, 2), o_part=f(K, MAX_SPLIT, HWb, DV),
                                             work=torch.zeros(4, dtype=torch.int32, device=p.eng.device), dec_in=f(K, HWb, DV))
        return self._mr

    def __getattr__(self, name):
        return getattr(self.plan, name)

    def grp(self, t, g):
        K = self.plan.obj_n
        return t[g * K:(g + 1) * K]

    def _build(self):
        p, qs, G = self.plan, self.qs, self.G
        K, N = p.obj_n, self.N
        D = p.eng.dec
        L = self.post
        grp = self.grp
        p._ws_cur, p._cnt_cur = p.ws, p.cnt
        d16, d8, d4, l2 = self.d16, self.d8, self.d4, self.l2
        for g in range(G):
            p._conv(L, D['convFM_m'], grp(self.dec_in, g), grp(d16[0], g), K, p.h16, p.w16, res=qs.fm_q[g:g + 1], res_mod=p.HW,
                    name='decoder.convFM.mem', lp_out='relu')
        p._resblock(L, D['ResMM'], d16[0], d16[1], d16[2], N, p.h16, p.w16, 'decoder.ResMM')
        for g in range(G):
            L.append(Launch(ops.upsample2x_add, (qs.s8[2][g:g + 1], grp(d16[2], g), grp(d8[0], g), True), 'decoder.RF3.up_add'))
        p._resblock(L, D['RF3']['ResMM'], d8[0], d8[1], d8[2], N, p.h8, p.w8, 'decoder.RF3.ResMM')
        for g in range(G):
            L.append(Launch(ops.upsample2x_add, (qs.s4[2][g:g + 1], grp(d8[2], g), grp(d4[0], g), True), 'decoder.RF2.up_add'))
        p._resblock(L, D['RF2']['ResMM'], d4[0], d4[1], d4[2], N, p.h4, p.w4, 'decoder.RF2.ResMM')
        p._conv(L, D['pred2'], d4[2], self.z4, N, p.h4, p.w4, relu_in=True, name='decoder.pred2.taps')
        L.append(Launch(ops.pred2_gather, (self.z4, D['pred2'].bias, self.pp), 'decoder.pred2.gather'))
        for g in range(G):
            L.append(Launch(ops.rough_uncertainty, (grp(self.pp, g), grp(self.p_up, g), grp(self.rough, g), self.unc[g]), 'decoder.rough_unc'))
            L.append(Launch(ops.local_stats, (qs.q['r1'][g], grp(self.rough, g), p.hs, p.hr, p.hm, grp(self.lm, g), grp(self.conf, g)),
                            'decoder.local_stats'))
            p._conv(L, D['local_convFM_loc'], grp(self.lm, g), grp(l2[0], g), K, p.h2, p.w2, res=qs.lq[g:g + 1],
                    res_mod=p.h2 * p.w2, name='decoder.local_convFM.local', lp_out='relu')
        p._resblock(L, D['local_ResMM'], l2[0], l2[1], l2[2], N, p.h2, p.w2, 'decoder.local_ResMM')
        p._conv(L, D['local_pred2'], l2[2], self.z2, N, p.h2, p.w2, relu_in=True, name='decoder.local_pred2.taps')
        L.append(Launch(ops.pred2_gather, (self.z2, D['local_pred2'].bias, self.qq), 'decoder.local_pred2.gather'))
        for g in range(G):
            L.append(Launch(ops.final_logits, (grp(self.p_up, g), self.unc[g], grp(self.conf, g), grp(self.qq, g), self.score[g:g + 1],
                                               p.pad, p.H0, p.W0), 'decoder.final_logits'))


class Engine:
    def __init__(self, model):
        dev = next(model.parameters()).device
        if dev.type != 'cuda':
            raise RuntimeError('AFB_URR runs on hand-written HIP kernels only: move the model to the GPU '
                               f'(model.to("cuda")); got {dev}.  There is no CPU fallback.')
        _lib.lib()
        self.device = dev
        self.model = model
        self.plans = {}
        self.precision = getattr(model, 'precision', 'fp32')
        if self.precision not in ops.MODES:
            raise ValueError(f"precision must be one of {sorted(ops.MODES)}, got {self.precision!r}")
        self.mode = ops.MODES[self.precision]
        pm = dict(getattr(model, 'precision_map', None) or {})
        for item in filter(None, os.environ.get('VFN_PRECISION_MAP', '').split(',')):
            k_, v_ = item.split('=')
            pm.setdefault(k_.strip(), v_.strip())
        for v_ in pm.values():
            if v_ not in ops.MODES:
                raise ValueError(f'precision map: unknown mode {v_!r}')
        self.pmap = sorted(((k_, ops.MODES[v_]) for k_, v_ in pm.items()), key=lambda kv: -len(kv[0]))
        self.mixed = bool(self.pmap)
        self.any_x3 = self.mode == 2 or any(m_ == 2 for _, m_ in self.pmap)
        self.fwd_count = 0
        self.mem_count = 0
        self.eager = False
        self._side = None
        self._side_busy = None
        from .refresh import Refresher
        self.refresher = Refresher(self.device)
        self._backward = None
        self._train_slot = 0
        self._batch = None
        self._pack(model)
        self._settle()

    def _settle(self):
        try:
            self.refresher.run()
        except RuntimeError:
            pass

    def refresh(self, check=True):
        self.refresher.run(verify=check)
        for layer in self._layers():
            if layer._w_lp:
                layer.refresh_derived()

    def _layers(self):
        def walk(o):
            if isinstance(o, (ConvLayer, Pred2Layer)):
                yield o
            elif isinstance(o, dict):
                for v in o.values():
                    yield from walk(v)
            elif isinstance(o, (list, tuple)):
                for v in o:
                    yield from walk(v)
        yield from walk([self.enc_q, self.enc_m, self.keyval, self.dec])

    def backward(self):
        from .backward import ModelBackward
        if self._backward is None:
            self._backward = ModelBackward(self)
            self._settle()
        self._backward.reset()
        return self._backward

    def use_winograd(self, layer, M, bf=0):
        if _WINOGRAD == '0' or getattr(layer, 'k', 0) != 3 or layer.stride != 1 or layer.pad != 1:
            return False
        if layer.cin % 32 or layer.cout % 4 or layer.cout < 32:
            return False
        if _WINOGRAD == '2':
            return True
        hit = (_WINO_TABLE_BF16.get((M, layer.cin, layer.cout)) if bf == 1 else None)
        if hit is None:
            hit = _WINO_TABLE.get((M, layer.cin, layer.cout))
        if hit is not None:
            return bool(hit)
        return layer.cin >= 128 and layer.cout >= 128 and M >= _WINOGRAD_MIN_M

    def winograd_tile(self, layer, M):
        if _WINOGRAD_F6 == '0':
            return 4
        if _WINOGRAD_F6 == '2':
            return 6
        return 6 if _WINOGRAD != '2' and _WINO_TABLE.get((M, layer.cin, layer.cout)) == 2 else 4

    def layer_mode(self, name):
        for prefix, m_ in self.pmap:
            if name.startswith(prefix):
                return m_
        return self.mode

    def layer_precision(self, name):
        return {v: k for k, v in ops.MODES.items()}[self.layer_mode(name)]

    def _pack_trunk(self, enc):
        dev = self.device
        out = {}
        for lname in ('res2', 'res3', 'res4'):
            blocks = []
            for blk in getattr(enc, lname):
                reg = self.refresher
                b = dict(conv1=ConvLayer(blk.conv1, blk.bn1, dev, reg=reg), conv2=ConvLayer(blk.conv2, blk.bn2, dev, reg=reg),
                         conv3=ConvLayer(blk.conv3, blk.bn3, dev, reg=reg))
# ... 450 lines not shown
```

v-floodnet_amd/ops.py:

```python
import ctypes as C
import os

import torch

from . import _lib
from ._lib import ptr, stream, check, ConvDesc


_cfg_tiles = None


def conv_cfg_tiles():
    global _cfg_tiles
    if _cfg_tiles is None:
        L = _lib.lib()
        out = []
        for c in range(L.vfn_conv_cfg_count()):
            bm, bn = C.c_int(), C.c_int()
            L.vfn_conv_cfg_tile(c, C.byref(bm), C.byref(bn))
            out.append((bm.value, bn.value))
        _cfg_tiles = tuple(out)
    return _cfg_tiles


def conv_cfg_wk(cfg):
    return _lib.lib().vfn_conv_cfg_wk(int(cfg))


def conv_cfg_tpb(cfg):
    return _lib.lib().vfn_conv_cfg_tpb(int(cfg))


def conv_cfgs(mode, _cache={}):
    mode = int(mode)
    if mode not in _cache:
        L = _lib.lib()
        _cache[mode] = tuple(c for c in range(L.vfn_conv_cfg_count()) if L.vfn_conv_cfg_modes(c) >> mode & 1)
    return _cache[mode]


def __getattr__(name):
    if name == 'BF16_CFGS':
        return conv_cfgs(1)
    raise AttributeError(f'module {__name__!r} has no attribute {name!r}')


def conv_cfg_kind(cfg):
    return _lib.lib().vfn_conv_cfg_kind(int(cfg))


SK_WS_FLOATS, SK_MAX_TILES = _lib.DEFINES['VFN_CONV_SK_WS_FLOATS'], _lib.DEFINES['VFN_CONV_SK_MAX_TILES']
_sk_scratch = {}


def streamk_scratch(device):
    key = str(device)
    if key not in _sk_scratch:
        _sk_scratch[key] = (torch.empty(SK_WS_FLOATS, dtype=torch.float32, device=device),
                            torch.zeros(SK_MAX_TILES, dtype=torch.int32, device=device))
    return _sk_scratch[key]


def set_streamk(desc, workspace, counters):
    assert workspace.numel() >= SK_WS_FLOATS and counters.numel() >= SK_MAX_TILES
    desc.ksplit, desc.split_from = 1, 0
    desc.partial, desc.tile_counters = ptr(workspace), ptr(counters)
    return desc


def conv_cfg_names(mode=0):
    L = _lib.lib()
    out = []
    for c in range(L.vfn_conv_cfg_count()):
        v = [C.c_int() for _ in range(5)]
        L.vfn_conv_cfg_info(c, *[C.byref(x) for x in v])
        bm, bn, wm, wn, dma = [x.value for x in v]
        wk, tpb = L.vfn_conv_cfg_wk(c), L.vfn_conv_cfg_tpb(c)
        if L.vfn_conv_cfg_kind(c) > 0:
            buf = C.create_string_buffer(96)
            L.vfn_conv_cfg_name(c, buf, 96)
            out.append(buf.value.decode())
            continue
        out.append(f'conv_igemm_dma_kernel<{bm}, {bn}, {wm}, {wn}, {dma}>' if dma else
                   f'conv_igemm_wk_kernel<{bm}, {bn}, {wm}, {wn}, {wk}, {4 if tpb > 1 else 3}, {tpb}, {int(mode)}>' if (wk > 1 or tpb > 1) else
                   f'conv_igemm_kernel<{bm}, {bn}, {wm}, {wn}, {int(mode)}>')
    return out


def pad_rows(wp, mult=256):
    cout = wp.shape[0]
    cp = (cout + mult - 1) // mult * mult
    if cp == cout:
        return wp.contiguous()
    out = torch.zeros(cp, wp.shape[1], dtype=wp.dtype, device=wp.device)
    out[:cout] = wp
    return out


def pack_weights_lp(wp, mode):
    if mode == 1:
        return wp.to(torch.bfloat16).contiguous()
    assert mode == 2 and wp.shape[1] % 32 == 0
    hi = wp.to(torch.bfloat16)
    lo = (wp - hi.float()).to(torch.bfloat16)
    cp, K = wp.shape
    return torch.cat([hi.view(cp, K // 32, 32), lo.view(cp, K // 32, 32)], dim=2).contiguous()


def make_conv_desc(x, wp, cout, kh, kw, stride, pad, out, scale=None, shift=None, res=None,
                   relu_in=False, relu_out=False, cin=None, in_ld=None, out_ld=None, res_ld=None,
                   N=None, H=None, W=None):
    if N is None:
        N, H, W = x.shape[0], x.shape[1], x.shape[2]
    in_ld = in_ld if in_ld is not None else x.shape[-1]
    cin = cin if cin is not None else in_ld
    Ho = (H + 2 * pad - kh) // stride + 1
    Wo = (W + 2 * pad - kw) // stride + 1
    out_ld = out_ld if out_ld is not None else out.shape[-1]
    d = ConvDesc()
    d.inp, d.w, d.scale, d.shift, d.res, d.out = ptr(x), ptr(wp), ptr(scale), ptr(shift), ptr(res), ptr(out)
    d.N, d.H, d.W, d.Cin, d.in_ld = N, H, W, cin, in_ld
    d.Ho, d.Wo, d.Cout, d.cout_pad = Ho, Wo, cout, wp.shape[0]
    d.out_ld = out_ld
    d.res_ld = res_ld if res_ld is not None else (res.shape[-1] if res is not None else 0)
    d.KH, d.KW, d.stride, d.pad = kh, kw, stride, pad
    d.relu_in, d.relu_out = int(relu_in), int(relu_out)
    d.M = N * Ho * Wo
    d.ksplit, d.split_from, d.partial = 1, 0, None
    d.tile_counters = None
    d.res_mod = 0
    d.w_packed = 0
    d.in_lp, d.out_lp_relu, d.out_lp = 0, 0, None
    d.mask, d.mask_ld, d.mask_after = None, 0, 0
    d.w_batch_rows = 0
    assert wp.shape[1] == kh * kw * cin
    return d


def use_packed_weights(desc, w_lp):
    desc.w = ptr(w_lp)
    desc.w_packed = 1
    return desc


def set_splitk(desc, ksplit, workspace, split_from=0, rows=None, counters=None):
    if ksplit > 1:
        rows = desc.M if rows is None else rows
        assert workspace is not None and workspace.numel() >= ksplit * rows * desc.Cout
        desc.ksplit, desc.split_from, desc.partial = int(ksplit), int(split_from), ptr(workspace)
        desc.tile_counters = ptr(counters) if counters is not None else None
    else:
        desc.ksplit, desc.split_from, desc.partial = 1, 0, None
        desc.tile_counters = None
    return desc


def tail_split_options(desc, bm, bn, max_split=8, mode=0):
    m_tiles = (desc.M + bm - 1) // bm
    n_tiles = (desc.Cout + bn - 1) // bn
    tiles = m_tiles * n_tiles
    out = []
    for unit in (256, 512):
        full = (tiles // unit) * unit
        full -= full % n_tiles
        if full <= 0 or full >= tiles:
            continue
        rows = desc.M - (full // n_tiles) * bm
        for ks in valid_splits(desc, max_split, mode)[1:]:
            out.append((full, ks, rows))
    return out


def valid_splits(desc, max_split=16, mode=0):
    nk = desc.KH * desc.KW * (desc.Cin // (64 if mode == 1 else 32))
    out = [1]
    if desc.Cout % 4 or desc.out_ld % 4 or (desc.res and desc.res_ld % 4):
        return out
    for s_ in range(2, max_split + 1):
        per = (nk + s_ - 1) // s_
        if per * (s_ - 1) < nk and per >= 4:
            out.append(s_)
    return out


MODES = {'fp32': 0, 'bf16': 1, 'bf16x3': 2}
_CONV_FN = ('vfn_conv2d_nhwc_f32', 'vfn_conv2d_nhwc_bf16', 'vfn_conv2d_nhwc_bf16x3')


WINO_GEMM_CFG0 = 1000
WINO_GEMM_TILES = ((128, 128, 4, 2), (64, 128, 2, 4), (128, 64, 4, 2), (64, 64, 2, 2))


def wino_gemm_cfg(tile_cfg, wgs=512):
    return WINO_GEMM_CFG0 + int(tile_cfg) + 8 * (int(wgs) // 128)


def wino_gemm_cfg_options(rows_pad, cout):
    out = []
    for tc in range(8):
        bm, bn = WINO_GEMM_TILES[tc & 3][:2]
        if rows_pad % bm or (bn > 64 and cout < 128):
            continue
        out += [wino_gemm_cfg(tc, w) for w in (256, 512, 768)]
    return out


PCONV_CFG0 = 2000


def pconv_cfg(tile_cfg, wgs=512):
    return PCONV_CFG0 + int(tile_cfg) + 8 * (int(wgs) // 128)


def pconv_eligible(desc, mode=0):
    lim = 0x7fffff00
    return (mode == 0 and desc.KH == 1 and desc.KW == 1 and desc.stride == 1 and desc.pad == 0 and not desc.mask and not desc.in_lp and
            not desc.out_lp and not desc.w_packed and not desc.w_batch_rows and desc.Cin % 32 == 0 and desc.in_ld % 4 == 0 and
            desc.M >= 1 and desc.M == desc.N * desc.H * desc.W and desc.M * desc.in_ld * 4 < lim and desc.M * desc.out_ld * 4 < lim and
            desc.cout_pad * desc.Cin * 4 < lim and
            (not desc.res or (desc.res_mod if desc.res_mod > 0 else desc.M) * desc.res_ld * 4 < lim))


def pconv_cfg_options(cout):
    out = []
    for tc in range(8):
        if WINO_GEMM_TILES[tc & 3][1] > 64 and cout < 128:
            continue
        out += [pconv_cfg(tc, w) for w in (256, 512, 768)]
    return out


def conv2d_launch(desc, cfg, mode=0):
    cfg = int(cfg)
    if cfg >= PCONV_CFG0:
        c = cfg - PCONV_CFG0
        if mode != 0:
            raise RuntimeError('the persistent 1x1 convolution is an f32 kernel')
        check(_lib.lib().vfn_conv1x1_persistent_f32(C.byref(desc), c & 7, (c >> 3) * 128, stream()), 'vfn_conv1x1_persistent_f32')
        return
    if cfg >= WINO_GEMM_CFG0:
        c, rows = cfg - WINO_GEMM_CFG0, desc.w_batch_rows
        if mode == 1 and rows > 0:
            check(_lib.lib().vfn_winograd_gemm_bf16(desc.inp, desc.w, desc.out, desc.M // rows, rows, desc.Cin, desc.Cout, desc.cout_pad, c & 7,
                                                    (c >> 3) * 128, stream()), 'vfn_winograd_gemm_bf16')
            return
        if mode != 0 or rows <= 0:
            raise RuntimeError('the persistent GEMM takes an f32 (or plain-bf16) Winograd-domain descriptor (w_batch_rows)')
        check(_lib.lib().vfn_winograd_gemm_f32(desc.inp, desc.w, desc.out, desc.M // rows, rows, desc.Cin, desc.Cout, desc.cout_pad, c & 7,
                                               (c >> 3) * 128, stream()), 'vfn_winograd_gemm_f32')
        return
    name = _CONV_FN[int(mode)]
    check(getattr(_lib.lib(), name)(C.byref(desc), cfg, stream()), name)


def conv_cfg_name(cfg, mode=0, _cache={}):
    cfg = int(cfg)
    if cfg >= WINO_GEMM_CFG0:
        c = (cfg - (PCONV_CFG0 if cfg >= PCONV_CFG0 else WINO_GEMM_CFG0)) & 7
        bm, bn, wm, wn = WINO_GEMM_TILES[c & 3]
        return f'wino_gemm_kernel<{bm}, {bn}, {wm}, {wn}, {1 + (c >> 2)}, {"true" if cfg >= PCONV_CFG0 else "false"}, {"true" if mode == 1 else "false"}>'
    if mode not in _cache:
        _cache[mode] = conv_cfg_names(mode)
    return _cache[mode][cfg]


def conv2d_nhwc(x, wp, cout, kh, kw, stride, pad, scale=None, shift=None, res=None,
                relu_in=False, relu_out=False, cfg=3, out=None, mode=0):
    N, H, W, _ = x.shape
    Ho = (H + 2 * pad - kh) // stride + 1
    Wo = (W + 2 * pad - kw) // stride + 1
    if out is None:
        out = torch.empty(N, Ho, Wo, cout, device=x.device, dtype=torch.float32)
    d = make_conv_desc(x, wp, cout, kh, kw, stride, pad, out, scale, shift, res, relu_in, relu_out)
    if mode == 0 and conv_cfg_kind(cfg) == 2:
        set_streamk(d, *streamk_scratch(x.device))
    conv2d_launch(d, cfg, mode)
    return out


_WINO_G = torch.tensor([[1 / 4, 0, 0], [-1 / 6, -1 / 6, -1 / 6], [-1 / 6, 1 / 6, -1 / 6], [1 / 24, 1 / 12, 1 / 6], [1 / 24, -1 / 12, 1 / 6], [0, 0, 1]],
                       dtype=torch.float64)
WINO_ROW_MULT = 256
_WINO_KROT = int(os.environ.get('VFN_KROT', '0'))


def pack_winograd_weight(w):
    cout, cin = w.shape[0], w.shape[1]
    assert tuple(w.shape[2:]) == (3, 3)
    g = w.detach().double().cpu()
    U = torch.einsum('ia,ocab,jb->ijoc', _WINO_G, g, _WINO_G)
    cp = (cout + 255) // 256 * 256
    out = torch.zeros(36, cp, cin, dtype=torch.float32)
    out[:, :cout] = U.reshape(36, cout, cin).float()
    return out.reshape(36 * cp, cin).contiguous()


def winograd_rows(N, H, W):
    t = N * ((H + 3) // 4) * ((W + 3) // 4)
    return (t + WINO_ROW_MULT - 1) // WINO_ROW_MULT * WINO_ROW_MULT


_WINO6_G = torch.tensor([[1, 0, 0], [-2 / 9, -2 / 9, -2 / 9], [-2 / 9, 2 / 9, -2 / 9], [1 / 90, 1 / 45, 2 / 45], [1 / 90, -1 / 45, 2 / 45],
                         [32 / 45, 16 / 45, 8 / 45], [32 / 45, -16 / 45, 8 / 45], [0, 0, 1]], dtype=torch.float64)
WINO6_ROW_MULT = 64


def pack_winograd6_weight(w):
    cout, cin = w.shape[0], w.shape[1]
    assert tuple(w.shape[2:]) == (3, 3)
    g, G = w.detach().double().cpu(), _WINO6_G
    col = lambda k: G[:, k].view(8, 1)
    tmp = (col(0) * g[:, :, None, 0, :] + col(1) * g[:, :, None, 1, :]) + col(2) * g[:, :, None, 2, :]
    U = (tmp[..., 0, None] * G[:, 0] + tmp[..., 1, None] * G[:, 1]) + tmp[..., 2, None] * G[:, 2]
    cp = (cout + 255) // 256 * 256
    out = torch.zeros(64, cp, cin, dtype=torch.float32)
    out[:, :cout] = U.permute(2, 3, 0, 1).reshape(64, cout, cin).float()
    return out.reshape(64 * cp, cin).contiguous()


def winograd6_tiles(N, H, W):
    return N * ((H + 5) // 6) * ((W + 5) // 6)


def winograd6_rows(N, H, W):
    return (winograd6_tiles(N, H, W) + WINO6_ROW_MULT - 1) // WINO6_ROW_MULT * WINO6_ROW_MULT


def pack_winograd_weight_bf16(w):
    return pack_winograd_weight(w).to(torch.bfloat16).contiguous()


def winograd_input(x, V, rows_pad, relu, N=None, H=None, W=None, cin=None, ld_x=None, tile=4):
    if N is None:
        N, H, W = x.shape[0], x.shape[1], x.shape[2]
    cin = cin if cin is not None else x.shape[-1]
    ld_x = ld_x if ld_x is not None else x.shape[-1]
    if tile == 6:
        check(_lib.lib().vfn_winograd6_input_f32(ptr(x), N, H, W, cin, ld_x, int(relu), ptr(V), rows_pad, stream()), 'vfn_winograd6_input_f32')
        return
    if V.dtype == torch.bfloat16:
        check(_lib.lib().vfn_winograd_input_bf16(ptr(x), N, H, W, cin, ld_x, int(relu), ptr(V), rows_pad, stream()), 'vfn_winograd_input_bf16')
        return
    check(_lib.lib().vfn_winograd_input_f32(ptr(x), N, H, W, cin, ld_x, int(relu), ptr(V), rows_pad, stream()), 'vfn_winograd_input_f32')


def winograd_output(Mb, rows_pad, out, N, H, W, cout, scale, shift, res, res_ld, res_mod, relu_out, out_ld=None, tile=4):
    name = 'vfn_winograd6_output_f32' if tile == 6 else 'vfn_winograd_output_f32'
    check(getattr(_lib.lib(), name)(ptr(Mb), rows_pad, N, H, W, cout, ptr(scale), ptr(shift), ptr(res), int(res_ld), int(res_mod),
                                    int(relu_out), ptr(out), out_ld if out_ld is not None else out.shape[-1], stream()), name)


def make_winograd_gemm_desc(V, U, Mb, rows_pad, cin, cout, comps=36):
    d = make_conv_desc(V, U, cout, 1, 1, 1, 0, Mb, None, None, None, False, False, cin=cin, in_ld=cin, out_ld=cout, N=1, H=1, W=comps * rows_pad)
    d.cout_pad = U.shape[0] // comps
    d.w_batch_rows = rows_pad
    d.k_rot = _WINO_KROT
    return d


def winograd_gemm(V, U, Mb, rows_pad, cin, cout, cfg=0, wgs=0, comps=36):
    check(_lib.lib().vfn_winograd_gemm_f32(ptr(V), ptr(U), ptr(Mb), comps, rows_pad, cin, cout, U.shape[0] // comps, int(cfg), int(wgs), stream()),
          'vfn_winograd_gemm_f32')


def conv2d_winograd(x, w, scale=None, shift=None, res=None, relu_in=False, relu_out=False, cfg=2, res_mod=0, tile=4):
    N, H, W, cin = x.shape
    cout = w.shape[0]
    if tile == 6:
        comps, rows, tiles = 64, winograd6_rows(N, H, W), winograd6_tiles(N, H, W)
        U = pack_winograd6_weight(w).to(x.device)
    else:
        comps, rows, tiles = 36, winograd_rows(N, H, W), vfn_winograd_tiles(N, H, W)
        U = pack_winograd_weight(w).to(x.device)
    V = torch.empty(comps * rows, cin, device=x.device, dtype=torch.float32)
    Mb = torch.empty(comps * rows, cout, device=x.device, dtype=torch.float32)
    out = torch.empty(N, H, W, cout, device=x.device, dtype=torch.float32)
    if rows > tiles and tile != 6:
        V.view(comps, rows, cin)[:, tiles:].zero_()
    winograd_input(x, V, rows, relu_in, tile=tile)
    d = make_winograd_gemm_desc(V, U, Mb, rows, cin, cout, comps)
    if conv_cfg_kind(cfg) == 2:
        set_streamk(d, *streamk_scratch(x.device))
    conv2d_launch(d, cfg, 0)
    winograd_output(Mb, rows, out, N, H, W, cout, scale, shift, res, res.shape[-1] if res is not None else 0, res_mod, relu_out, tile=tile)
    return out


def vfn_winograd_tiles(N, H, W):
    return N * ((H + 3) // 4) * ((W + 3) // 4)


def make_stem_desc(frame, mask, w, scale, shift, out, mean, std, N, H0, W0, pad, Hp, Wp):
    from ._lib import StemDesc
    d = StemDesc()
    d.frame, d.mask, d.w, d.scale, d.shift, d.out = ptr(frame), ptr(mask), ptr(w), ptr(scale), ptr(shift), ptr(out)
    for i in range(3):
        d.mean[i] = float(mean[i])
        d.std[i] = float(std[i])
    d.N, d.cin = N, (5 if mask is not None else 3)
    d.H0, d.W0 = H0, W0
    d.pad_top, d.pad_left = pad[2], pad[0]
    d.Hp, d.Wp, d.Ho, d.Wo = Hp, Wp, Hp // 2, Wp // 2
    return d


def stem_launch(desc):
    check(_lib.lib().vfn_stem_conv7x7_f32(C.byref(desc), stream()), 'vfn_stem_conv7x7_f32')


def pack_stem_weight(ws):
    w = torch.cat([x.detach().float() for x in ws], dim=1)
    P = w.shape[1]
    out = torch.zeros(P, 7, 8, 64, dtype=torch.float32, device=w.device)
    out[:, :, :7, :] = w.permute(1, 2, 3, 0)
    return out.reshape(P * 56, 64).contiguous()


def maxpool3x3s2(x, out):
    N, H, W, Cc = x.shape
    check(_lib.lib().vfn_maxpool3x3s2_nhwc_f32(ptr(x), ptr(out), N, H, W, Cc, stream()), 'vfn_maxpool3x3s2_nhwc_f32')
    return out


def upsample2x_add(s, pm, out, s_bcast, out_lp=None, lp_relu=False):
    N, h, w, Cc = out.shape
    if out_lp is not None:
        check(_lib.lib().vfn_upsample2x_add_lp_nhwc_f32(ptr(s), ptr(pm), ptr(out), ptr(out_lp), int(lp_relu), N, h, w, Cc,
                                                        int(s_bcast), stream()), 'vfn_upsample2x_add_lp_nhwc_f32')
        return out
    check(_lib.lib().vfn_upsample2x_add_nhwc_f32(ptr(s), ptr(pm), ptr(out), N, h, w, Cc, int(s_bcast), stream()),
          'vfn_upsample2x_add_nhwc_f32')
    return out


def rough_uncertainty(p, p_up, rough, unc):
    obj_n, h, w, _ = p.shape
    check(_lib.lib().vfn_rough_uncertainty_f32(ptr(p), ptr(p_up), ptr(rough), ptr(unc), obj_n, h, w, stream()),
          'vfn_rough_uncertainty_f32')


def local_stats(r1, rough, hs, hr, hm, lm, conf):
    obj_n, h, w = rough.shape
    Cc = r1.shape[-1]
    L = _lib.lib()
    if Cc == 64 and obj_n <= 4:
        check(L.vfn_local_stats_f32(ptr(r1), ptr(rough), ptr(lm), ptr(conf), obj_n, h, w, Cc, stream()), 'vfn_local_stats_f32')
        return
    check(L.vfn_local_hpass_f32(ptr(r1), ptr(rough), ptr(hs), ptr(hr), ptr(hm), obj_n, h, w, Cc, stream()),
          'vfn_local_hpass_f32')
    check(L.vfn_local_vpass_f32(ptr(hs), ptr(hr), ptr(hm), ptr(lm), ptr(conf), obj_n, h, w, Cc, stream()),
          'vfn_local_vpass_f32')


def local_stats_two_pass(r1, rough, hs, hr, hm, lm, conf):
    obj_n, h, w = rough.shape
    Cc = r1.shape[-1]
    L = _lib.lib()
    check(L.vfn_local_hpass_f32(ptr(r1), ptr(rough), ptr(hs), ptr(hr), ptr(hm), obj_n, h, w, Cc, stream()), 'vfn_local_hpass_f32')
    check(L.vfn_local_vpass_f32(ptr(hs), ptr(hr), ptr(hm), ptr(lm), ptr(conf), obj_n, h, w, Cc, stream()), 'vfn_local_vpass_f32')


def pred2_gather(z, bias, out):
    N, h, w, ldz = z.shape
    check(_lib.lib().vfn_pred2_gather_f32(ptr(z), ptr(bias), ptr(out), N, h, w, ldz, stream()), 'vfn_pred2_gather_f32')
    return out


def final_logits(p_up, unc, conf, q, score, pad, H0, W0):
    obj_n, h, w, _ = p_up.shape
    check(_lib.lib().vfn_final_logits_f32(ptr(p_up), ptr(unc), ptr(conf), ptr(q), ptr(score), obj_n, h, w,
                                          pad[2], pad[0], H0, W0, stream()), 'vfn_final_logits_f32')


def segment_uncertainty(score):
    bs, obj_n, H, W = score.shape
    assert score.is_contiguous()
    partial = torch.empty(bs * 64, device=score.device, dtype=torch.float32)
    out = torch.empty(1, device=score.device, dtype=torch.float32)
    check(_lib.lib().vfn_segment_uncertainty_f32(ptr(score), bs, obj_n, H * W, ptr(partial), ptr(out), stream()),
          'vfn_segment_uncertainty_f32')
    return out[0]


def segment_loss(score, label, lu, want_grad=True):
    bs, obj_n, H, W = score.shape
    assert score.is_contiguous()
    lab = label.to(device=score.device, dtype=torch.int32).contiguous()
    partial = torch.empty(2 * bs * 64, device=score.device, dtype=torch.float32)
    stats = torch.empty(3 + bs, device=score.device, dtype=torch.float32)
    grad = torch.empty_like(score) if want_grad else None
    check(_lib.lib().vfn_segment_loss_f32(ptr(score), ptr(lab), bs, obj_n, H * W, float(lu), ptr(partial), ptr(stats), ptr(grad),
                                          stream()), 'vfn_segment_loss_f32')
    return stats, grad


_wgrad_ws = {}
_WGRAD_INLAUNCH = os.environ.get('VFN_WGRAD_INLAUNCH', '0') == '1'
_STEM_WGRAD = os.environ.get('VFN_STEM_WGRAD', '1') == '1'


def conv_wgrad(x, gy, k, stride, pad, cin=None, cout=None, ld_x=None, relu=False, rowscale=None, out=None, accumulate=False,
               N=None, H=None, W=None, ksplit=None, batch=1, x_bstride=0, g_bstride=0):
    from ._lib import WgradDesc
    if N is None:
        N, H, W = x.shape[0], x.shape[1], x.shape[2]
    Ho, Wo = gy.shape[1], gy.shape[2]
    ld_x = ld_x if ld_x is not None else (x.stride(-2) if x.dim() >= 2 else x.shape[-1])
    cin = cin if cin is not None else x.shape[-1]
    cout = cout if cout is not None else gy.shape[-1]
    ld_g = gy.stride(-2)
    assert x.stride(-1) == 1 and gy.stride(-1) == 1
    Kc = k * k * cin
    if out is None:
        assert not accumulate
        out = torch.empty(cout, Kc, device=x.device, dtype=torch.float32)
    assert out.is_contiguous() and out.numel() == batch * cout * Kc
    M = N * Ho * Wo
    if (_STEM_WGRAD and k == 7 and stride == 2 and pad == 3 and cout == 64 and cin in (3, 5) and ld_x == cin and ld_g == 64 and batch == 1
            and not relu and ksplit is None and Ho == (H - 1) // 2 + 1 and Wo == (W - 1) // 2 + 1):
        L = _lib.lib()
        key = (str(x.device), torch.cuda.current_stream(x.device).cuda_stream, 'stem')
        need = L.vfn_stem_wgrad_scratch_floats(cin)
        part = _wgrad_ws.get(key)
        if part is None or part.numel() < need:
            part = _wgrad_ws[key] = torch.empty(need, device=x.device, dtype=torch.float32)
        check(L.vfn_stem_wgrad_f32(ptr(x), ptr(gy), ptr(rowscale), ptr(out), ptr(part), part.numel(), N, H, W, cin, Ho, Wo, int(accumulate),
                                   stream()), 'vfn_stem_wgrad_f32')
        return out
    tiles = ((cout + 63) // 64 if cout > 32 else 1) * k * k * ((cin + (31 if cin <= 32 else 63)) // (32 if cin <= 32 else 64))
    tiles *= batch
    if ksplit is None:
        ksplit = max(1, min(64, 2048 // tiles, M // 300))
        if batch == 1 and cin > 32:
            ksplit = max(1, min(64, M // 300, max((256 + tiles - 1) // tiles, M // 800)))
    d = WgradDesc()
    d.x, d.gy, d.rowscale, d.dw = ptr(x), ptr(gy), ptr(rowscale), ptr(out)
    d.N, d.H, d.W, d.Cin, d.ld_x = N, H, W, cin, ld_x
    d.Ho, d.Wo, d.Cout, d.ld_g = Ho, Wo, cout, ld_g
    d.k, d.stride, d.pad, d.relu, d.accumulate, d.ksplit = k, stride, pad, int(relu), int(accumulate), int(ksplit)
    d.batch, d.x_bstride, d.g_bstride = int(batch), int(x_bstride), int(g_bstride)
    part = None
    if ksplit > 1:
        key = (str(x.device), torch.cuda.current_stream(x.device).cuda_stream)
        need = batch * ksplit * cout * Kc
        hit = _wgrad_ws.get(key)
        if hit is None or hit[0].numel() < need:
            hit = (torch.empty(max(need, 8 * 1024 * 1024), device=x.device, dtype=torch.float32),
                   hit[1] if hit is not None else torch.zeros(16384, dtype=torch.int32, device=x.device))
            _wgrad_ws[key] = hit
        part = hit[0]
        if _WGRAD_INLAUNCH and tiles <= hit[1].numel() and need * 4 < 0x7fffff00:
            d.tile_counters = ptr(hit[1])
    d.partial = ptr(part)
    check(_lib.lib().vfn_conv_wgrad_f32(C.byref(d), stream()), 'vfn_conv_wgrad_f32')
    return out


def winograd_gy(gy, Z, rows_pad, N, H, W, cout, ld_g):
    check(_lib.lib().vfn_winograd_gy_f32(ptr(gy), N, H, W, cout, ld_g, ptr(Z), rows_pad, stream()), 'vfn_winograd_gy_f32')


_wino_wgrad_ws = {}

# ... 327 lines not shown
```

Measured before the change: 166.1.

## Fuse bottleneck downsample shortcut into conv3 GEMM and add 32-row Winograd tiles

```diff
diff --git a/include/vfn_shortcut_fused.h b/include/vfn_shortcut_fused.h
--- /dev/null
+++ b/include/vfn_shortcut_fused.h
@@ -0,0 +1,14 @@
+#ifndef VFN_SHORTCUT_FUSED_H
+#define VFN_SHORTCUT_FUSED_H
+
+#ifdef __cplusplus
+extern "C" {
+#endif
+
+int vfn_conv1x1_shortcut_fused_f32(const vfn_conv_desc* sc, const vfn_conv_desc* main_layer, int cfg, int wgs, void* stream);
+
+#ifdef __cplusplus
+}
+#endif
+
+#endif
diff --git a/v-floodnet_amd/_lib.py b/v-floodnet_amd/_lib.py
--- a/v-floodnet_amd/_lib.py
+++ b/v-floodnet_amd/_lib.py
@@ -17,8 +17,8 @@
 _DECLARATOR = re.compile(r'(?:const\s+)?([A-Za-z_][\w ]*?)(?:\s*(\*)\s*|\s+)(\w+)\s*(?:\[([^\]]*)\])?')
 
 
-def parse_header(text):
-    defines, enums, structs, protos = {}, {}, {}, {}
+def parse_header(text, known_structs=None):
+    defines, enums, structs, protos = {}, {}, dict(known_structs or {}), {}
 
     def fail(why, decl):
         raise RuntimeError(f'vfn_hip.h: {why}: {" ".join(decl.split())[:120]!r}')
@@ -112,7 +112,7 @@
             protos[m.group(1)] = [] if params == 'void' else [declarator(p, decl, True)[1] for p in params.split(',')]
             continue
         fail('declaration not understood', decl)
-    return defines, enums, structs, protos
+    return defines, enums, {k: v for k, v in structs.items() if k not in (known_structs or {})}, protos
 
 
 with open(os.path.join(os.path.dirname(_HERE), 'include', 'vfn_hip.h')) as _f:
@@ -122,6 +122,8 @@
     SIGNATURES_WINOGRAD6 = parse_header(_f.read())[3]
 with open(os.path.join(os.path.dirname(_HERE), 'include', 'vfn_image_val.h')) as _f:
     DEFINES_IMAGE_VAL, _, _, SIGNATURES_IMAGE_VAL = parse_header(_f.read())
+with open(os.path.join(os.path.dirname(_HERE), 'include', 'vfn_shortcut_fused.h')) as _f:
+    SIGNATURES_SHORTCUT_FUSED = parse_header(_f.read(), STRUCTS)[3]
 SEG_SCORES_CHUNK, SEG_SCORES_MAX_BLOCKS = DEFINES_IMAGE_VAL['VFN_SEG_SCORES_CHUNK'], DEFINES_IMAGE_VAL['VFN_SEG_SCORES_MAX_BLOCKS']
 ABI_VERSION = DEFINES['VFN_ABI_VERSION']
 TRAIN_AUG_MAX_T, TRAIN_AUG_MAX_SIDE, TRAIN_AUG_MAX_OUT, TRAIN_AUG_MAX_OBJ = (
@@ -176,6 +178,8 @@
             declare(name, SIGNATURES_WINOGRAD6, 'vfn_winograd6.h')
         for name in SIGNATURES_IMAGE_VAL:
             declare(name, SIGNATURES_IMAGE_VAL, 'vfn_image_val.h')
+        for name in SIGNATURES_SHORTCUT_FUSED:
+            declare(name, SIGNATURES_SHORTCUT_FUSED, 'vfn_shortcut_fused.h')
         _lib = L
     return _lib
 
diff --git a/v-floodnet_amd/csrc/conv_winograd.hip b/v-floodnet_amd/csrc/conv_winograd.hip
--- a/v-floodnet_amd/csrc/conv_winograd.hip
+++ b/v-floodnet_amd/csrc/conv_winograd.hip
@@ -2,6 +2,7 @@
 #include "conv_internal.h"
 #include "../../include/vfn_hip.h"
 #include "../../include/vfn_winograd6.h"
+#include "../../include/vfn_shortcut_fused.h"
 
 namespace {
 
@@ -417,229 +418,36 @@
     const float* res;
 };
 
+struct wino_dual_args {
+    const float* V;
+    const float* U;
+    const float* scale;
+    const float* shift;
+    int C, a_ld, cout_pad, relu_in, relu_mid, stride, H, W, Ho, Wo, pix;
+};
+
 template <int BM, int BN, int WM, int WN, int PD, bool CONV = false, bool LP = false>
 __global__ __launch_bounds__(WM * WN * 64)
 void wino_gemm_kernel(const wino_gemm_args p) {
-    static_assert(!(CONV && LP), "the reduced-precision form is the transform-domain GEMM only");
-    constexpr int BK = 32;
-    constexpr int KT = LP ? 64 : 32;
-    constexpr int ES = LP ? 2 : 4;
-    constexpr int NT = WM * WN * 64;
-    constexpr int TM = BM / WM / 32, TN = BN / WN / 32;
-    constexpr int AC = BM * 8 / NT, BC = BN * 8 / NT, RSTEP = NT / 8;
-    static_assert(AC >= 1 && BC >= 1, "tile too small for the thread count");
-    extern __shared__ __attribute__((aligned(16))) char smem[];
-    float* sA = reinterpret_cast<float*>(smem);
-    float* sB = sA + 2 * BM * BK;
-
-    const int tid = threadIdx.x, lane = tid & 63, wave = tid >> 6;
-    const int wm = wave / WN, wn = wave % WN;
-    const int li = lane & 31, lh = lane >> 5;
-
-    const int per = p.mtiles * p.ntiles, total = p.comps * per;
-    const int gx = (int)gridDim.x >> 3, xcd = (int)blockIdx.x & 7, loc = (int)blockIdx.x >> 3;
-    const int q = total >> 3, r8 = total & 7;
-    const int u_begin = xcd < r8 ? xcd * (q + 1) : r8 * (q + 1) + (xcd - r8) * q;
-    const int u_end = u_begin + q + (xcd < r8 ? 1 : 0);
-    const int first = u_begin + loc;
-    const int n_units = first < u_end ? (u_end - first + gx - 1) / gx : 0;
-    const int nk = p.C / KT;
-    const int T = n_units * nk;
-    if (T == 0) return;
-
-    const int c16 = tid & 7, r0 = tid >> 3;
-    const int a_ld = CONV ? p.a_ld : p.C;
-    const __amdgpu_buffer_rsrc_t rsV = __builtin_amdgcn_make_buffer_rsrc(const_cast<float*>(p.V), 0, (int)((size_t)p.comps * p.rows_pad * a_ld * ES), 0x00020000);
-    const __amdgpu_buffer_rsrc_t rsU = __builtin_amdgcn_make_buffer_rsrc(const_cast<float*>(p.U), 0, (int)((size_t)p.comps * p.cout_pad * p.C * ES), 0x00020000);
-    int a_thr[AC], b_thr[BC];
-#pragma unroll
-    for (int j = 0; j < AC; ++j) a_thr[j] = (r0 + j * RSTEP) * a_ld * ES + c16 * 16;
-#pragma unroll
-    for (int j = 0; j < BC; ++j) b_thr[j] = (r0 + j * RSTEP) * p.C * ES + c16 * 16;
-
-    int lu = 0, lkt = 0, la_base = 0, lb_base = 0;
-    int n0_cur = 0;
-    auto unit_bases = [&](int ui, int& a_base, int& b_base, size_t& o_base, int* n0 = nullptr) {
-        const int u = first + ui * gx;
-        const int xi = u / per, rem = u - xi * per;
-        const int mt = rem / p.ntiles, nt = rem - mt * p.ntiles;
-        a_base = (xi * p.rows_pad + mt * BM) * a_ld * ES;
-        b_base = (xi * p.cout_pad + nt * BN) * p.C * ES;
-        o_base = CONV ? (size_t)mt * BM : ((size_t)xi * p.rows_pad + mt * BM) * p.Cout + nt * BN;
-        if (n0) *n0 = nt * BN;
-    };
-    size_t o_dummy;
-    unit_bases(0, la_base, lb_base, o_dummy);
-    f32x4 ra[PD][AC], rb[PD][BC];
-    auto request = [&](int slot) {
-        const int koff = lkt * 128;
-#pragma unroll
-        for (int j = 0; j < AC; ++j)
-            ra[slot][j] = __builtin_bit_cast(f32x4, __builtin_amdgcn_raw_buffer_load_b128(rsV, a_thr[j], la_base + koff, 0));
-#pragma unroll
-        for (int j = 0; j < BC; ++j)
-            rb[slot][j] = __builtin_bit_cast(f32x4, __builtin_amdgcn_raw_buffer_load_b128(rsU, b_thr[j], lb_base + koff, 0));
-        if (++lkt == nk) {
-            lkt = 0;
-            if (++lu < n_units) unit_bases(lu, la_base, lb_base, o_dummy);
-        }
-    };
-    const float relu_floor = (CONV && p.relu_in) ? 0.f : -INFINITY;
-    auto stage = [&](int buf, int slot) {
-        float* dA = sA + buf * BM * BK;
-        float* dB = sB + buf * BN * BK;
-#pragma unroll
-        for (int j = 0; j < AC; ++j) {
-            const int r = r0 + j * RSTEP;
-            f32x4 v = ra[slot][j];
-            if constexpr (CONV) {
-#pragma unroll
-                for (int e = 0; e < 4; ++e) v[e] = fmaxf(v[e], relu_floor);
-            }
-            *reinterpret_cast<f32x4*>(dA + r * BK + ((c16 ^ ((r >> 1) & 7)) << 2)) = v;
-        }
-#pragma unroll
-        for (int j = 0; j < BC; ++j) {
-            const int r = r0 + j * RSTEP;
-            *reinterpret_cast<f32x4*>(dB + r * BK + ((c16 ^ ((r >> 1) & 7)) << 2)) = rb[slot][j];
-        }
-    };
-
-    f32x16 acc[TM][TN];
-#pragma unroll
-    for (int i = 0; i < TM; ++i)
-#pragma unroll
-        for (int j = 0; j < TN; ++j)
-#pragma unroll
-            for (int r = 0; r < 16; ++r) acc[i][j][r] = 0.f;
-
-    int cu = 0, ckt = 0, ca_dummy, cb_dummy;
-    size_t o_base;
-    unit_bases(0, ca_dummy, cb_dummy, o_base, &n0_cur);
-
-#pragma unroll
-    for (int d = 0; d < PD; ++d)
-        if (d < T) request(d);
-    stage(0, 0);
-    __syncthreads();
-
-    for (int t0 = 0; t0 < T; t0 += PD) {
-#pragma unroll
-        for (int uu = 0; uu < PD; ++uu) {
-            const int t = t0 + uu;
-            if (t >= T) break;
-            const int buf = t & 1;
-            const bool more = t + 1 < T;
-            const bool more_req = t + PD < T;
-            const float* cA = sA + buf * BM * BK + (wm * TM * 32) * BK;
-            const float* cB = sB + buf * BN * BK + (wn * TN * 32) * BK;
-            auto read_frags = [&](int kk, f32x4 (&a)[TM], f32x4 (&b)[TN]) {
-                const int lc = 2 * kk + lh;
-#pragma unroll
-                for (int i = 0; i < TM; ++i) {
-                    const int r = i * 32 + li;
-                    a[i] = *reinterpret_cast<const f32x4*>(cA + r * BK + ((lc ^ ((r >> 1) & 7)) << 2));
-                }
-#pragma unroll
-                for (int j = 0; j < TN; ++j) {
-                    const int r = j * 32 + li;
-                    b[j] = *reinterpret_cast<const f32x4*>(cB + r * BK + ((lc ^ ((r >> 1) & 7)) << 2));
-                }
-            };
-            f32x4 fa[2][TM], fb[2][TN];
-            read_frags(0, fa[0], fb[0]);
-#pragma unroll
-            for (int kk = 0; kk < 4; ++kk) {
-                if (PD > 1 && kk == 0 && more) stage(buf ^ 1, (uu + 1) % PD);
-                if (kk == 1 && more_req) request(uu);
-                if (PD == 1 && kk == 3 && more) stage(buf ^ 1, 0);
-                if (kk + 1 < 4) read_frags(kk + 1, fa[(kk + 1) & 1], fb[(kk + 1) & 1]);
-                if constexpr (LP) {
-                    typedef __attribute__((ext_vector_type(8))) __bf16 bf16x8_;
-#pragma unroll
-                    for (int i = 0; i < TM; ++i)
-#pragma unroll
-                        for (int j = 0; j < TN; ++j)
-                            acc[i][j] = __builtin_amdgcn_mfma_f32_32x32x16_bf16(__builtin_bit_cast(bf16x8_, fa[kk & 1][i]), __builtin_bit_cast(bf16x8_, fb[kk & 1][j]),
-                                                                                acc[i][j], 0, 0, 0);
-                } else {
-#pragma unroll
-                for (int e = 0; e < 4; ++e)
-#pragma unroll
-                    for (int i = 0; i < TM; ++i)
-#pragma unroll
-                        for (int j = 0; j < TN; ++j)
-                            acc[i][j] = __builtin_amdgcn_mfma_f32_32x32x2f32(fa[kk & 1][i][e], fb[kk & 1][j][e], acc[i][j], 0, 0, 0);
-                }
-            }
-            if (++ckt == nk) {
-                if constexpr (CONV) {
-                    const int m0 = (int)o_base;
-                    const int npix = p.rows_pad;
-                    const __amdgpu_buffer_rsrc_t rso = __builtin_amdgcn_make_buffer_rsrc(p.Mb, 0, (int)((size_t)npix * p.out_ld * 4), 0x00020000);
-                    const __amdgpu_buffer_rsrc_t rsr = __builtin_amdgcn_make_buffer_rsrc(const_cast<float*>(p.res ? p.res : p.V), 0,
-                        p.res ? (int)((size_t)(p.res_mod > 0 ? p.res_mod : npix) * p.res_ld * 4) : 0, 0x00020000);
-                    const float floor_ = p.relu_out ? 0.f : -INFINITY;
-                    float rv[TM][TN][16];
-#pragma unroll
-                    for (int j = 0; j < TN; ++j) {
-                        const int col = n0_cur + (wn * TN + j) * 32 + li;
-#pragma unroll
-                        for (int i = 0; i < TM; ++i)
-#pragma unroll
-                            for (int r = 0; r < 16; ++r) {
-                                const int row = m0 + (wm * TM + i) * 32 + 4 * lh + (r & 3) + 8 * (r >> 2);
-                                const int rrow = p.res_mod > 0 ? row % p.res_mod : row;
-                                rv[i][j][r] = __builtin_bit_cast(float, __builtin_amdgcn_raw_buffer_load_b32(
-                                    rsr, (row < npix && col < p.Cout) ? (rrow * p.res_ld + col) * 4 : 0x7ffffff0, 0, 0));
-                            }
-                    }
-#pragma unroll
-                    for (int j = 0; j < TN; ++j) {
-                        const int col = n0_cur + (wn * TN + j) * 32 + li;
-                        const bool cok = col < p.Cout;
-                        const float sc = (p.scale && cok) ? p.scale[col] : 1.f;
-                        const float sh = (p.shift && cok) ? p.shift[col] : 0.f;
-#pragma unroll
-                        for (int i = 0; i < TM; ++i)
-#pragma unroll
-                            for (int r = 0; r < 16; ++r) {
-                                const int row = m0 + (wm * TM + i) * 32 + 4 * lh + (r & 3) + 8 * (r >> 2);
-                                const float v = vfn_floor_nan(acc[i][j][r] * sc + sh + rv[i][j][r], floor_);
-                                __builtin_amdgcn_raw_buffer_store_b32(__builtin_bit_cast(unsigned, v), rso,
-                                                                      (row < npix && cok) ? (row * p.out_ld + col) * 4 : 0x7ffffff0, 0, 0);
-                                acc[i][j][r] = 0.f;
-                            }
-                    }
-                } else {
-                float* o = p.Mb + o_base;
-#pragma unroll
-                for (int j = 0; j < TN; ++j) {
-                    const int col = (wn * TN + j) * 32 + li;
-#pragma unroll
-                    for (int i = 0; i < TM; ++i) {
-                        const int rbase = (wm * TM + i) * 32 + 4 * lh;
-#pragma unroll
-                        for (int r = 0; r < 16; ++r) {
-                            if (n0_cur + col < p.Cout)
-                                o[(size_t)(rbase + (r & 3) + 8 * (r >> 2)) * p.Cout + col] = acc[i][j][r];
-                            acc[i][j][r] = 0.f;
-                        }
-                    }
-                }
-                }
-                ckt = 0;
-                if (++cu < n_units) unit_bases(cu, ca_dummy, cb_dummy, o_base, &n0_cur);
-            }
-            __syncthreads();
-        }
-    }
-}
-
-template <int BM, int BN, int WM, int WN, int PD, bool CONV, bool LP>
-int launch_wino_gemm(const wino_gemm_args& a, int wgs, hipStream_t s) {
+    constexpr bool DUAL = false;
+    constexpr wino_dual_args q2{};
+#include "wino_gemm_body.inc"
+}
+
+template <int BM, int BN, int WM, int WN, int PD>
+__global__ __launch_bounds__(WM * WN * 64)
+void wino_gemm_dual_kernel(const wino_gemm_args p, const wino_dual_args q2) {
+    constexpr bool DUAL = true, CONV = true, LP = false;
+#include "wino_gemm_body.inc"
+}
+
+template <int BM, int BN, int WM, int WN, int PD, bool CONV, bool LP, bool DUAL = false>
+int launch_wino_gemm(const wino_gemm_args& a, int wgs, hipStream_t s, const wino_dual_args* dual = nullptr) {
     constexpr size_t lds = 2 * (size_t)(BM + BN) * 32 * sizeof(float);
-    static const bool lds_ready = vfn_allow_lds(&wino_gemm_kernel<BM, BN, WM, WN, PD, CONV, LP>, lds);
+    static const bool lds_ready = [] {
+        if constexpr (DUAL) return vfn_allow_lds(&wino_gemm_dual_kernel<BM, BN, WM, WN, PD>, lds);
+        else return vfn_allow_lds(&wino_gemm_kernel<BM, BN, WM, WN, PD, CONV, LP>, lds);
+    }();
     (void)lds_ready;
     wino_gemm_args p = a;
     p.mtiles = (a.rows_pad + BM - 1) / BM;
@@ -648,20 +456,41 @@
     int grid = wgs > 0 ? wgs : 512;
     if (grid > total) grid = total;
     grid = (grid + 7) / 8 * 8;
-    hipLaunchKernelGGL((wino_gemm_kernel<BM, BN, WM, WN, PD, CONV, LP>), dim3(grid), dim3(WM * WN * 64), lds, s, p);
+    if constexpr (DUAL)
+        hipLaunchKernelGGL((wino_gemm_dual_kernel<BM, BN, WM, WN, PD>), dim3(grid), dim3(WM * WN * 64), lds, s, p, *dual);
+    else
+        hipLaunchKernelGGL((wino_gemm_kernel<BM, BN, WM, WN, PD, CONV, LP>), dim3(grid), dim3(WM * WN * 64), lds, s, p);
     return vfn_check_launch();
 }
 
 constexpr int kWinoTile[4][4] = {{128, 128, 4, 2}, {64, 128, 2, 4}, {128, 64, 4, 2}, {64, 64, 2, 2}};
 constexpr int kWinoCfgs = 8;
 
-template <bool CONV, bool LP>
-int launch_wino_cfg(const wino_gemm_args& a, int cfg, int wgs, hipStream_t s) {
-    return vfn_dispatch<kWinoCfgs>(cfg, [&](auto id) -> int {
+constexpr int kWinoDualCfgs = 4;
+
+template <bool CONV, bool LP, bool DUAL = false>
+int launch_wino_cfg(const wino_gemm_args& a, int cfg, int wgs, hipStream_t s, const wino_dual_args* dual = nullptr) {
+    return vfn_dispatch<DUAL ? kWinoDualCfgs : kWinoCfgs>(cfg, [&](auto id) -> int {
         constexpr int c = decltype(id)::value;
         constexpr const int* t = kWinoTile[c & 3];
-        return launch_wino_gemm<t[0], t[1], t[2], t[3], 1 + (c >> 2), CONV, LP>(a, wgs, s);
+        return launch_wino_gemm<t[0], t[1], t[2], t[3], 1 + (c >> 2), CONV, LP, DUAL>(a, wgs, s, dual);
     });
+}
+
+constexpr int kWinoTile32[2][4] = {{32, 128, 1, 4}, {32, 64, 1, 2}};
+constexpr int kWinoCfgs32 = 8;
+
+inline const int* wino_tile_of(int cfg) { return cfg < kWinoCfgs ? kWinoTile[cfg & 3] : kWinoTile32[cfg & 1]; }
+inline bool wino_cfg32_ok(int cfg) { return cfg >= kWinoCfgs && cfg < kWinoCfgs + kWinoCfgs32 && (cfg & 3) < 2; }
+
+int launch_wino_cfg32(const wino_gemm_args& a, int cfg, int wgs, hipStream_t s) {
+    switch (cfg - kWinoCfgs) {
+        case 0: return launch_wino_gemm<32, 128, 1, 4, 1, false, false>(a, wgs, s);
+        case 1: return launch_wino_gemm<32, 64, 1, 2, 1, false, false>(a, wgs, s);
+        case 4: return launch_wino_gemm<32, 128, 1, 4, 2, false, false>(a, wgs, s);
+        case 5: return launch_wino_gemm<32, 64, 1, 2, 2, false, false>(a, wgs, s);
+    }
+    return VFN_ERR_ARG;
 }
 
 inline bool tensors_fit_32bit(int N, int H, int W, int ld, int res_ld, int mask_ld, int res_mod) {
@@ -751,11 +580,13 @@
 
 extern "C" int vfn_winograd_gemm_f32(const float* V, const float* U, float* Mb, int comps, int rows_pad, int C, int Cout, int cout_pad, int cfg,
                                      int wgs, void* stream) {
-    if (!V || !U || !Mb || comps < 1 || rows_pad < 1 || C < 32 || C % 32 || Cout < 1 || cout_pad < Cout || cfg < 0 || cfg >= kWinoCfgs) return VFN_ERR_ARG;
-    const int bm = kWinoTile[cfg & 3][0], bn = kWinoTile[cfg & 3][1];
+    if (!V || !U || !Mb || comps < 1 || rows_pad < 1 || C < 32 || C % 32 || Cout < 1 || cout_pad < Cout || cfg < 0 ||
+        (cfg >= kWinoCfgs && !wino_cfg32_ok(cfg))) return VFN_ERR_ARG;
+    const int bm = wino_tile_of(cfg)[0], bn = wino_tile_of(cfg)[1];
     if (rows_pad % bm || cout_pad < (Cout + bn - 1) / bn * bn) return VFN_ERR_ARG;
     if ((long long)comps * rows_pad * C * 4 >= 0x7fffff00LL || (long long)comps * cout_pad * C * 4 >= 0x7fffff00LL) return VFN_ERR_ARG;
     wino_gemm_args a{V, U, Mb, comps, rows_pad, C, Cout, cout_pad, 0, 0, 0, 0, 0, 0, 0, 0, nullptr, nullptr, nullptr};
+    if (cfg >= kWinoCfgs) return launch_wino_cfg32(a, cfg, wgs, (hipStream_t)stream);
     return launch_wino_cfg<false, false>(a, cfg, wgs, (hipStream_t)stream);
 }
 
@@ -773,6 +604,27 @@
     return launch_wino_cfg<true, false>(a, cfg, wgs, (hipStream_t)stream);
 }
 
+extern "C" int vfn_conv1x1_shortcut_fused_f32(const vfn_conv_desc* sc, const vfn_conv_desc* d, int cfg, int wgs, void* stream) {
+    if (!sc || !d || !sc->in || !sc->w || !d->in || !d->w || !d->out || cfg < 0 || cfg >= kWinoDualCfgs) return VFN_ERR_ARG;
+    for (const vfn_conv_desc* l : {sc, d})
+        if (l->KH != 1 || l->KW != 1 || l->pad != 0 || l->mask || l->in_lp || l->out_lp || l->w_packed || l->ksplit > 1 || l->w_batch_rows ||
+            l->res || l->Cin < 32 || l->Cin % 32 || l->in_ld < l->Cin || l->in_ld % 4 || l->N < 1 || l->H < 1 || l->W < 1) return VFN_ERR_ARG;
+    if (d->stride != 1 || (sc->stride != 1 && sc->stride != 2)) return VFN_ERR_ARG;
+    if (d->M < 1 || d->M != d->N * d->H * d->W || sc->Ho != (sc->H - 1) / sc->stride + 1 || sc->Wo != (sc->W - 1) / sc->stride + 1 ||
+        sc->M != sc->N * sc->Ho * sc->Wo || sc->M != d->M || sc->Cout != d->Cout || d->Cout < 1 || d->out_ld < d->Cout) return VFN_ERR_ARG;
+    const int bn = kWinoTile[cfg & 3][1];
+    const int need = (d->Cout + bn - 1) / bn * bn;
+    if (d->cout_pad < need || sc->cout_pad < need) return VFN_ERR_ARG;
+    const long long lim = 0x7fffff00LL, pix2 = (long long)sc->N * sc->H * sc->W;
+    if (pix2 * sc->in_ld * 4 >= lim || (long long)d->M * d->in_ld * 4 >= lim || (long long)d->M * d->out_ld * 4 >= lim ||
+        (long long)d->cout_pad * d->Cin * 4 >= lim || (long long)sc->cout_pad * sc->Cin * 4 >= lim) return VFN_ERR_ARG;
+    wino_gemm_args a{d->in, d->w, d->out, 1, d->M, d->Cin, d->Cout, d->cout_pad, 0, 0,
+                     d->in_ld, d->out_ld, 0, 0, d->relu_in, d->relu_out, d->scale, d->shift, nullptr};
+    const wino_dual_args a2{sc->in, sc->w, sc->scale, sc->shift, sc->Cin, sc->in_ld, sc->cout_pad, sc->relu_in, sc->relu_out, sc->stride,
+                            sc->H, sc->W, sc->Ho, sc->Wo, (int)pix2};
+    return launch_wino_cfg<true, false, true>(a, cfg, wgs, (hipStream_t)stream, &a2);
+}
+
 extern "C" int vfn_winograd_input_bf16(const float* x, int N, int H, int W, int C, int ld_x, int relu, void* V, int rows_pad, void* stream) {
     if (!x || !V || N < 1 || H < 1 || W < 1 || C < 4 || C % 4 || ld_x < C || ld_x % 4 || rows_pad < vfn_winograd_tiles(N, H, W)) return VFN_ERR_ARG;
     const long long total = (long long)vfn_winograd_tiles(N, H, W) * (C / 4);
diff --git a/v-floodnet_amd/csrc/wino_gemm_body.inc b/v-floodnet_amd/csrc/wino_gemm_body.inc
--- /dev/null
+++ b/v-floodnet_amd/csrc/wino_gemm_body.inc
@@ -0,0 +1,293 @@
+    static_assert(!(CONV && LP), "the reduced-precision form is the transform-domain GEMM only");
+    static_assert(CONV || !DUAL, "two sources: the 1x1 convolution form only");
+    constexpr int BK = 32;
+    constexpr int KT = LP ? 64 : 32;
+    constexpr int ES = LP ? 2 : 4;
+    constexpr int NT = WM * WN * 64;
+    constexpr int TM = BM / WM / 32, TN = BN / WN / 32;
+    constexpr int AC = BM * 8 / NT, BC = BN * 8 / NT, RSTEP = NT / 8;
+    static_assert(AC >= 1 && BC >= 1, "tile too small for the thread count");
+    extern __shared__ __attribute__((aligned(16))) char smem[];
+    float* sA = reinterpret_cast<float*>(smem);
+    float* sB = sA + 2 * BM * BK;
+
+    const int tid = threadIdx.x, lane = tid & 63, wave = tid >> 6;
+    const int wm = wave / WN, wn = wave % WN;
+    const int li = lane & 31, lh = lane >> 5;
+
+    const int per = p.mtiles * p.ntiles, total = p.comps * per;
+    const int gx = (int)gridDim.x >> 3, xcd = (int)blockIdx.x & 7, loc = (int)blockIdx.x >> 3;
+    const int q = total >> 3, r8 = total & 7;
+    const int u_begin = xcd < r8 ? xcd * (q + 1) : r8 * (q + 1) + (xcd - r8) * q;
+    const int u_end = u_begin + q + (xcd < r8 ? 1 : 0);
+    const int first = u_begin + loc;
+    const int n_units = first < u_end ? (u_end - first + gx - 1) / gx : 0;
+    const int nkA = DUAL ? q2.C / KT : 0;
+    const int nk = p.C / KT + nkA;
+    const int T = n_units * nk;
+    if (T == 0) return;
+
+    const int c16 = tid & 7, r0 = tid >> 3;
+    const int a_ld = CONV ? p.a_ld : p.C;
+    const __amdgpu_buffer_rsrc_t rsV = __builtin_amdgcn_make_buffer_rsrc(const_cast<float*>(p.V), 0, (int)((size_t)p.comps * p.rows_pad * a_ld * ES), 0x00020000);
+    const __amdgpu_buffer_rsrc_t rsU = __builtin_amdgcn_make_buffer_rsrc(const_cast<float*>(p.U), 0, (int)((size_t)p.comps * p.cout_pad * p.C * ES), 0x00020000);
+    int a_thr[AC], b_thr[BC];
+#pragma unroll
+    for (int j = 0; j < AC; ++j) a_thr[j] = (r0 + j * RSTEP) * a_ld * ES + c16 * 16;
+#pragma unroll
+    for (int j = 0; j < BC; ++j) b_thr[j] = (r0 + j * RSTEP) * p.C * ES + c16 * 16;
+
+    int lu = 0, lkt = 0, la_base = 0, lb_base = 0;
+    __amdgpu_buffer_rsrc_t rsV2 = rsV, rsU2 = rsU;
+    int a_thr2[AC], b_thr2[BC], lb2_base = 0;
+    float rfloor[PD];
+    if constexpr (DUAL) {
+        rsV2 = __builtin_amdgcn_make_buffer_rsrc(const_cast<float*>(q2.V), 0, (int)((size_t)q2.pix * q2.a_ld * 4), 0x00020000);
+        rsU2 = __builtin_amdgcn_make_buffer_rsrc(const_cast<float*>(q2.U), 0, (int)((size_t)q2.cout_pad * q2.C * 4), 0x00020000);
+#pragma unroll
+        for (int j = 0; j < BC; ++j) b_thr2[j] = (r0 + j * RSTEP) * q2.C * 4 + c16 * 16;
+    }
+    auto unit_dual = [&](int ui) {
+        if constexpr (DUAL) {
+            const int u = first + ui * gx;
+            const int mt = u / p.ntiles, nt = u - mt * p.ntiles;
+            lb2_base = nt * BN * q2.C * 4;
+            const int hw = q2.Ho * q2.Wo;
+#pragma unroll
+            for (int j = 0; j < AC; ++j) {
+                const int row = mt * BM + r0 + j * RSTEP;
+                const int n = row / hw, rem = row - n * hw;
+                const int yo = rem / q2.Wo, xo = rem - yo * q2.Wo;
+                a_thr2[j] = row < p.rows_pad ? ((n * q2.H + q2.stride * yo) * q2.W + q2.stride * xo) * q2.a_ld * 4 + c16 * 16 : 0x7fffff00;
+            }
+        }
+    };
+    int n0_cur = 0;
+    auto unit_bases = [&](int ui, int& a_base, int& b_base, size_t& o_base, int* n0 = nullptr) {
+        const int u = first + ui * gx;
+        const int xi = u / per, rem = u - xi * per;
+        const int mt = rem / p.ntiles, nt = rem - mt * p.ntiles;
+        a_base = (xi * p.rows_pad + mt * BM) * a_ld * ES;
+        b_base = (xi * p.cout_pad + nt * BN) * p.C * ES;
+        o_base = CONV ? (size_t)mt * BM : ((size_t)xi * p.rows_pad + mt * BM) * p.Cout + nt * BN;
+        if (n0) *n0 = nt * BN;
+    };
+    size_t o_dummy;
+    unit_bases(0, la_base, lb_base, o_dummy);
+    if constexpr (DUAL) unit_dual(0);
+    f32x4 ra[PD][AC], rb[PD][BC];
+    auto request = [&](int slot) {
+        if constexpr (DUAL) {
+            if (lkt < nkA) {
+                const int koff = lkt * 128;
+#pragma unroll
+                for (int j = 0; j < AC; ++j)
+                    ra[slot][j] = __builtin_bit_cast(f32x4, __builtin_amdgcn_raw_buffer_load_b128(rsV2, a_thr2[j], koff, 0));
+#pragma unroll
+                for (int j = 0; j < BC; ++j)
+                    rb[slot][j] = __builtin_bit_cast(f32x4, __builtin_amdgcn_raw_buffer_load_b128(rsU2, b_thr2[j], lb2_base + koff, 0));
+                rfloor[slot] = q2.relu_in ? 0.f : -INFINITY;
+            } else {
+                const int koff = (lkt - nkA) * 128;
+#pragma unroll
+                for (int j = 0; j < AC; ++j)
+                    ra[slot][j] = __builtin_bit_cast(f32x4, __builtin_amdgcn_raw_buffer_load_b128(rsV, a_thr[j], la_base + koff, 0));
+#pragma unroll
+                for (int j = 0; j < BC; ++j)
+                    rb[slot][j] = __builtin_bit_cast(f32x4, __builtin_amdgcn_raw_buffer_load_b128(rsU, b_thr[j], lb_base + koff, 0));
+                rfloor[slot] = p.relu_in ? 0.f : -INFINITY;
+            }
+            if (++lkt == nk) {
+                lkt = 0;
+                if (++lu < n_units) {
+                    unit_bases(lu, la_base, lb_base, o_dummy);
+                    unit_dual(lu);
+                }
+            }
+            return;
+        }
+        const int koff = lkt * 128;
+#pragma unroll
+        for (int j = 0; j < AC; ++j)
+            ra[slot][j] = __builtin_bit_cast(f32x4, __builtin_amdgcn_raw_buffer_load_b128(rsV, a_thr[j], la_base + koff, 0));
+#pragma unroll
+        for (int j = 0; j < BC; ++j)
+            rb[slot][j] = __builtin_bit_cast(f32x4, __builtin_amdgcn_raw_buffer_load_b128(rsU, b_thr[j], lb_base + koff, 0));
+        if (++lkt == nk) {
+            lkt = 0;
+            if (++lu < n_units) unit_bases(lu, la_base, lb_base, o_dummy);
+        }
+    };
+    const float relu_floor = (CONV && p.relu_in) ? 0.f : -INFINITY;
+    auto stage = [&](int buf, int slot) {
+        float* dA = sA + buf * BM * BK;
+        float* dB = sB + buf * BN * BK;
+#pragma unroll
+        for (int j = 0; j < AC; ++j) {
+            const int r = r0 + j * RSTEP;
+            f32x4 v = ra[slot][j];
+            if constexpr (CONV) {
+#pragma unroll
+                for (int e = 0; e < 4; ++e) v[e] = fmaxf(v[e], DUAL ? rfloor[slot] : relu_floor);
+            }
+            *reinterpret_cast<f32x4*>(dA + r * BK + ((c16 ^ ((r >> 1) & 7)) << 2)) = v;
+        }
+#pragma unroll
+        for (int j = 0; j < BC; ++j) {
+            const int r = r0 + j * RSTEP;
+            *reinterpret_cast<f32x4*>(dB + r * BK + ((c16 ^ ((r >> 1) & 7)) << 2)) = rb[slot][j];
+        }
+    };
+
+    f32x16 acc[TM][TN];
+#pragma unroll
+    for (int i = 0; i < TM; ++i)
+#pragma unroll
+        for (int j = 0; j < TN; ++j)
+#pragma unroll
+            for (int r = 0; r < 16; ++r) acc[i][j][r] = 0.f;
+
+    f32x16 keep[DUAL ? TM : 1][DUAL ? TN : 1];
+    int cu = 0, ckt = 0, ca_dummy, cb_dummy;
+    size_t o_base;
+    unit_bases(0, ca_dummy, cb_dummy, o_base, &n0_cur);
+
+#pragma unroll
+    for (int d = 0; d < PD; ++d)
+        if (d < T) request(d);
+    stage(0, 0);
+    __syncthreads();
+
+    for (int t0 = 0; t0 < T; t0 += PD) {
+#pragma unroll
+        for (int uu = 0; uu < PD; ++uu) {
+            const int t = t0 + uu;
+            if (t >= T) break;
+            const int buf = t & 1;
+            const bool more = t + 1 < T;
+            const bool more_req = t + PD < T;
+            const float* cA = sA + buf * BM * BK + (wm * TM * 32) * BK;
+            const float* cB = sB + buf * BN * BK + (wn * TN * 32) * BK;
+            auto read_frags = [&](int kk, f32x4 (&a)[TM], f32x4 (&b)[TN]) {
+                const int lc = 2 * kk + lh;
+#pragma unroll
+                for (int i = 0; i < TM; ++i) {
+                    const int r = i * 32 + li;
+                    a[i] = *reinterpret_cast<const f32x4*>(cA + r * BK + ((lc ^ ((r >> 1) & 7)) << 2));
+                }
+#pragma unroll
+                for (int j = 0; j < TN; ++j) {
+                    const int r = j * 32 + li;
+                    b[j] = *reinterpret_cast<const f32x4*>(cB + r * BK + ((lc ^ ((r >> 1) & 7)) << 2));
+                }
+            };
+            f32x4 fa[2][TM], fb[2][TN];
+            read_frags(0, fa[0], fb[0]);
+#pragma unroll
+            for (int kk = 0; kk < 4; ++kk) {
+                if (PD > 1 && kk == 0 && more) stage(buf ^ 1, (uu + 1) % PD);
+                if (kk == 1 && more_req) request(uu);
+                if (PD == 1 && kk == 3 && more) stage(buf ^ 1, 0);
+                if (kk + 1 < 4) read_frags(kk + 1, fa[(kk + 1) & 1], fb[(kk + 1) & 1]);
+                if constexpr (LP) {
+                    typedef __attribute__((ext_vector_type(8))) __bf16 bf16x8_;
+#pragma unroll
+                    for (int i = 0; i < TM; ++i)
+#pragma unroll
+                        for (int j = 0; j < TN; ++j)
+                            acc[i][j] = __builtin_amdgcn_mfma_f32_32x32x16_bf16(__builtin_bit_cast(bf16x8_, fa[kk & 1][i]), __builtin_bit_cast(bf16x8_, fb[kk & 1][j]),
+                                                                                acc[i][j], 0, 0, 0);
+                } else {
+#pragma unroll
+                for (int e = 0; e < 4; ++e)
+#pragma unroll
+                    for (int i = 0; i < TM; ++i)
+#pragma unroll
+                        for (int j = 0; j < TN; ++j)
+                            acc[i][j] = __builtin_amdgcn_mfma_f32_32x32x2f32(fa[kk & 1][i][e], fb[kk & 1][j][e], acc[i][j], 0, 0, 0);
+                }
+            }
+            if constexpr (DUAL) {
+                if (ckt + 1 == nkA) {
+                    const float floor2 = q2.relu_mid ? 0.f : -INFINITY;
+#pragma unroll
+                    for (int j = 0; j < TN; ++j) {
+                        const int col = n0_cur + (wn * TN + j) * 32 + li;
+                        const bool cok = col < p.Cout;
+                        const float sc = (q2.scale && cok) ? q2.scale[col] : 1.f;
+                        const float sh = (q2.shift && cok) ? q2.shift[col] : 0.f;
+#pragma unroll
+                        for (int i = 0; i < TM; ++i)
+#pragma unroll
+                            for (int r = 0; r < 16; ++r) {
+                                keep[i][j][r] = vfn_floor_nan(acc[i][j][r] * sc + sh, floor2);
+                                acc[i][j][r] = 0.f;
+                            }
+                    }
+                }
+            }
+            if (++ckt == nk) {
+                if constexpr (CONV) {
+                    const int m0 = (int)o_base;
+                    const int npix = p.rows_pad;
+                    const __amdgpu_buffer_rsrc_t rso = __builtin_amdgcn_make_buffer_rsrc(p.Mb, 0, (int)((size_t)npix * p.out_ld * 4), 0x00020000);
+                    const __amdgpu_buffer_rsrc_t rsr = __builtin_amdgcn_make_buffer_rsrc(const_cast<float*>(p.res ? p.res : p.V), 0,
+                        p.res ? (int)((size_t)(p.res_mod > 0 ? p.res_mod : npix) * p.res_ld * 4) : 0, 0x00020000);
+                    const float floor_ = p.relu_out ? 0.f : -INFINITY;
+                    float rv[TM][TN][16];
+#pragma unroll
+                    for (int j = 0; j < TN; ++j) {
+                        if constexpr (DUAL) break;
+                        const int col = n0_cur + (wn * TN + j) * 32 + li;
+#pragma unroll
+                        for (int i = 0; i < TM; ++i)
+#pragma unroll
+                            for (int r = 0; r < 16; ++r) {
+                                const int row = m0 + (wm * TM + i) * 32 + 4 * lh + (r & 3) + 8 * (r >> 2);
+                                const int rrow = p.res_mod > 0 ? row % p.res_mod : row;
+                                rv[i][j][r] = __builtin_bit_cast(float, __builtin_amdgcn_raw_buffer_load_b32(
+                                    rsr, (row < npix && col < p.Cout) ? (rrow * p.res_ld + col) * 4 : 0x7ffffff0, 0, 0));
+                            }
+                    }
+#pragma unroll
+                    for (int j = 0; j < TN; ++j) {
+                        const int col = n0_cur + (wn * TN + j) * 32 + li;
+                        const bool cok = col < p.Cout;
+                        const float sc = (p.scale && cok) ? p.scale[col] : 1.f;
+                        const float sh = (p.shift && cok) ? p.shift[col] : 0.f;
+#pragma unroll
+                        for (int i = 0; i < TM; ++i)
+#pragma unroll
+                            for (int r = 0; r < 16; ++r) {
+                                const int row = m0 + (wm * TM + i) * 32 + 4 * lh + (r & 3) + 8 * (r >> 2);
+                                float res_v;
+                                if constexpr (DUAL) res_v = keep[i][j][r]; else res_v = rv[i][j][r];
+                                const float v = vfn_floor_nan(acc[i][j][r] * sc + sh + res_v, floor_);
+                                __builtin_amdgcn_raw_buffer_store_b32(__builtin_bit_cast(unsigned, v), rso,
+                                                                      (row < npix && cok) ? (row * p.out_ld + col) * 4 : 0x7ffffff0, 0, 0);
+                                acc[i][j][r] = 0.f;
+                            }
+                    }
+                } else {
+                float* o = p.Mb + o_base;
+#pragma unroll
+                for (int j = 0; j < TN; ++j) {
+                    const int col = (wn * TN + j) * 32 + li;
+#pragma unroll
+                    for (int i = 0; i < TM; ++i) {
+                        const int rbase = (wm * TM + i) * 32 + 4 * lh;
+#pragma unroll
+                        for (int r = 0; r < 16; ++r) {
+                            if (n0_cur + col < p.Cout)
+                                o[(size_t)(rbase + (r & 3) + 8 * (r >> 2)) * p.Cout + col] = acc[i][j][r];
+                            acc[i][j][r] = 0.f;
+                        }
+                    }
+                }
+                }
+                ckt = 0;
+                if (++cu < n_units) unit_bases(cu, ca_dummy, cb_dummy, o_base, &n0_cur);
+            }
+            __syncthreads();
+        }
+    }
diff --git a/v-floodnet_amd/engine.py b/v-floodnet_amd/engine.py
--- a/v-floodnet_amd/engine.py
+++ b/v-floodnet_amd/engine.py
@@ -21,6 +21,8 @@
 _TABLE_PATHS = (_TUNED_PATH, _TUNED_BF16_PATH, _TUNED_BF16X3_PATH)
 _TUNED_WINO6 = {}
 _TUNED_WINO6_PATH = _TUNED_PATH.replace('tuned_gfx950.json', 'tuned_gfx950_wino6.json')
+_TUNED_SHORTCUT = {}
+_TUNED_SHORTCUT_PATH = _TUNED_PATH.replace('tuned_gfx950.json', 'tuned_gfx950_shortcut.json')
 
 
 def is_wino6_desc(d):
@@ -44,12 +46,19 @@
             for k, v in json.load(open(path)).items():
                 t = (int(v[0]), int(v[1]), int(v[2]) if len(v) > 2 else 0)
                 table[tuple(int(x) for x in k.split(','))] = t + tuple(int(x) for x in v[3:6]) if len(v) >= 6 else t
+    path = _TUNED_SHORTCUT_PATH
+    alt = os.environ.get('VFN_TUNED_DIR')
+    if alt and os.path.isfile(os.path.join(alt, os.path.basename(path))):
+        path = os.path.join(alt, os.path.basename(path))
+    if os.path.isfile(path):
+        for k, v in json.load(open(path)).items():
+            _TUNED_SHORTCUT[tuple(int(x) for x in k.split(','))] = (int(v[0]), int(v[1]))
 
 
 def save_tuned(path=None, mode=0):
     import json
-    table = _TUNED_WINO6 if mode == 'wino6' else _TABLES[mode]
-    with open(path or (_TUNED_WINO6_PATH if mode == 'wino6' else _TABLE_PATHS[mode]), 'w') as f:
+    table = _TUNED_WINO6 if mode == 'wino6' else _TUNED_SHORTCUT if mode == 'shortcut' else _TABLES[mode]
+    with open(path or (_TUNED_WINO6_PATH if mode == 'wino6' else _TUNED_SHORTCUT_PATH if mode == 'shortcut' else _TABLE_PATHS[mode]), 'w') as f:
         json.dump({','.join(str(x) for x in k): list(v) for k, v in sorted(table.items())}, f, indent=0)
 
 
@@ -73,6 +82,8 @@
 _TRAIN_SLOTS = int(os.environ.get('VFN_TRAIN_SLOTS', 2))
 _WINOGRAD = os.environ.get('VFN_WINOGRAD', '1')
 _WINOGRAD_F6 = os.environ.get('VFN_WINOGRAD_F6', '1')
+_WINO_ROWS32 = os.environ.get('VFN_WINO_ROWS32', '1')
+_SHORTCUT_FUSED = os.environ.get('VFN_SHORTCUT_FUSED', '1')
 _WINOGRAD_LP = os.environ.get('VFN_WINOGRAD_LP', '1') == '1'
 _WINOGRAD_MIN_M = int(os.environ.get('VFN_WINOGRAD_MIN_M', 10000))
 _WINO_TABLE = {}
@@ -183,7 +194,7 @@
 
     best, best_t = None, None
     if d.w_batch_rows > 0 and bf == 1:
-        for c in ops.wino_gemm_cfg_options(d.w_batch_rows, d.Cout):
+        for c in ops.wino_gemm_cfg_options(d.w_batch_rows, d.Cout, rows32=False):
             if cfg_filter is not None and not cfg_filter(key, c):
                 continue
             t = timeit(c)
@@ -191,7 +202,7 @@
                 best, best_t = (c, 1, 0), t
         return best
     if d.w_batch_rows > 0 and bf == 0 and d.M // d.w_batch_rows * d.w_batch_rows == d.M:
-        for c in ops.wino_gemm_cfg_options(d.w_batch_rows, d.Cout):
+        for c in ops.wino_gemm_cfg_options(d.w_batch_rows, d.Cout, rows32=False):
             if cfg_filter is not None and not cfg_filter(key, c):
                 continue
             apply_choice(d, (c, 1, 0), ws, cnt)
@@ -592,6 +603,11 @@
     def _conv_winograd(self, lst, layer, x, out, N, H, Wd, res, relu_in, relu_out, name, out_ld, res_mod, bf=0, tile=4):
         comps = 64 if tile == 6 else 36
         rows = ops.winograd6_rows(N, H, Wd) if tile == 6 else ops.winograd_rows(N, H, Wd)
+        if tile == 6 and bf == 0 and _WINO_ROWS32 != '0':
+            rows32 = (ops.winograd6_tiles(N, H, Wd) + 31) // 32 * 32
+            c32 = _TUNED_WINO6.get((64 * rows32, layer.cout, layer.cin))
+            if rows32 < rows and (_WINO_ROWS32 == '2' or (c32 is not None and ops.is_wino_gemm32_cfg(c32[0]))):
+                rows = rows32
         key = id(self._ws_cur)
         need_v, need_m = comps * rows * layer.cin, comps * rows * layer.cout
         V, Mb = self._wino.get(key, (None, None))
@@ -617,7 +633,8 @@
         elif tile == 6:
             choice = _TUNED_WINO6.get((dg.M, layer.cout, layer.cin))
             if choice is None or choice[0] not in ops.wino_gemm_cfg_options(rows, layer.cout):
-                choice = (ops.wino_gemm_cfg(5 if layer.cout >= 128 else 7, 768), 1, 0)
+                choice = ((ops.wino_gemm32_cfg(4 if layer.cout >= 128 else 5, 768) if rows % 64 else
+                           ops.wino_gemm_cfg(5 if layer.cout >= 128 else 7, 768)), 1, 0)
         else:
             choice = choose_cfg(dg.M, layer.cout, layer.cin, 0)
         cfg = apply_choice(dg, choice, self._ws_cur, self._cnt_cur)
@@ -647,21 +664,48 @@
                 self._conv(lst, blk['conv1'], x, t1, N, H, Wd, relu_out=True, name=nm + '.conv1', lp_out='plain', f32_out=False)
                 self._conv(lst, blk['conv2'], t1, t2, N, H, Wd, relu_out=True, name=nm + '.conv2', lp_out='plain',
                            f32_out=False)
-                if 'down' in blk:
+                out = lb['out'] if bi == len(blocks) - 1 else lb['o'][bi % 2]
+                if self.keep_acts and bi != len(blocks) - 1:
+                    out = torch.empty_like(out)
+                if 'down' in blk and self._shortcut_fused(lst, blk, x, t2, out, N, H, Wd, Ho, Wo, nm):
+                    idn = None
+                elif 'down' in blk:
                     self._conv(lst, blk['down'], x, ds_buf, N, H, Wd, name=nm + '.down')
                     idn = ds_buf
                 else:
                     idn = x
-                out = lb['out'] if bi == len(blocks) - 1 else lb['o'][bi % 2]
-                if self.keep_acts and bi != len(blocks) - 1:
-                    out = torch.empty_like(out)
-                self._conv(lst, blk['conv3'], t2, out, N, Ho, Wo, res=idn, relu_out=True, name=nm + '.conv3',
-                           lp_out='plain')
+                if idn is not None:
+                    self._conv(lst, blk['conv3'], t2, out, N, Ho, Wo, res=idn, relu_out=True, name=nm + '.conv3',
+                               lp_out='plain')
                 if self.keep_acts and acts is not None:
                     acts[(lname, bi)] = dict(x=x, t1=t1, t2=t2, ds=ds_buf if 'down' in blk else None, out=out, stride=s, H=H, W=Wd)
                 x = out
                 H, Wd = Ho, Wo
         return x
+
+    def _shortcut_fused(self, lst, blk, x, t2, out, N, H, Wd, Ho, Wo, nm):
+        down, conv3 = blk['down'], blk['conv3']
+        if (_SHORTCUT_FUSED == '0' or self.keep_acts or self.eng.layer_mode(nm + '.down') != 0 or self.eng.layer_mode(nm + '.conv3') != 0 or
+                x.shape[-1] != down.cin or t2.shape[-1] != conv3.cin):
+            return False
+        sc = ops.make_conv_desc(x, down.w, down.cout, down.k, down.k, down.stride, down.pad, None, down.scale, down.shift,
+                                cin=down.cin, out_ld=down.cout, N=N, H=H, W=Wd)
+        d = ops.make_conv_desc(t2, conv3.w, conv3.cout, conv3.k, conv3.k, conv3.stride, conv3.pad, out, conv3.scale, conv3.shift,
+                               relu_out=True, cin=conv3.cin, N=N, H=Ho, W=Wo)
+        if not ops.shortcut_fused_eligible(sc, d, 0):
+            return False
+        options = ops.shortcut_fused_cfg_options(sc, d)
+        choice = _TUNED_SHORTCUT.get((d.M, d.Cout, sc.Cin, d.Cin))
+        if choice is not None and choice[0] < 0:
+            return False
+        if choice is None or tuple(choice) not in options:
+            choice = (1 if d.Cout >= 128 else 3, 768)
+            if choice not in options:
+                return False
+        self._lp_state.pop((out.data_ptr(), tuple(out.shape)), None)
+        lst.append(Launch(ops.shortcut_fused_launch, (sc, d, choice[0], choice[1]),
+                          f'{nm}.down+conv3[{d.M}x{d.Cout}x{sc.Cin}+{d.M}x{d.Cout}x{d.Cin}]', 2.0 * d.M * d.Cout * (sc.Cin + d.Cin)))
+        return True
 
     def _resblock(self, lst, rb, x, t, out, N, H, Wd, name):
         self._conv(lst, rb['conv1'], x, t, N, H, Wd, relu_in=True, name=name + '.conv1', lp_out='relu', f32_out=False)
diff --git a/v-floodnet_amd/ops.py b/v-floodnet_amd/ops.py
--- a/v-floodnet_amd/ops.py
+++ b/v-floodnet_amd/ops.py
@@ -195,13 +195,38 @@
     return WINO_GEMM_CFG0 + int(tile_cfg) + 8 * (int(wgs) // 128)
 
 
-def wino_gemm_cfg_options(rows_pad, cout):
+WINO_GEMM32_CFG0 = 1500
+WINO_GEMM_TILES32 = ((32, 128, 1, 4), (32, 64, 1, 2))
+
+
+def wino_gemm32_cfg(tile_cfg, wgs=512):
+    assert (int(tile_cfg) & 3) < len(WINO_GEMM_TILES32) and 0 <= int(tile_cfg) < 8
+    return WINO_GEMM32_CFG0 + int(tile_cfg) + 8 * (int(wgs) // 128)
+
+
+def is_wino_gemm32_cfg(cfg):
+    return WINO_GEMM32_CFG0 <= int(cfg) < PCONV_CFG0
+
+
+def persistent_cfg_info(cfg):
+    cfg = int(cfg)
+    c = cfg - (PCONV_CFG0 if cfg >= PCONV_CFG0 else WINO_GEMM32_CFG0 if cfg >= WINO_GEMM32_CFG0 else WINO_GEMM_CFG0)
+    tiles = WINO_GEMM_TILES32 if is_wino_gemm32_cfg(cfg) else WINO_GEMM_TILES
+    return tuple(tiles[c & 3]) + (1 + ((c & 7) >> 2), (c >> 3) * 128)
+
+
+def wino_gemm_cfg_options(rows_pad, cout, rows32=True):
     out = []
     for tc in range(8):
         bm, bn = WINO_GEMM_TILES[tc & 3][:2]
         if rows_pad % bm or (bn > 64 and cout < 128):
             continue
         out += [wino_gemm_cfg(tc, w) for w in (256, 512, 768)]
+    for tc in (0, 1, 4, 5) if rows32 else ():
+        bm, bn = WINO_GEMM_TILES32[tc & 3][:2]
+        if rows_pad % bm or (bn > 64 and cout < 128):
+            continue
+        out += [wino_gemm32_cfg(tc, w) for w in (256, 512, 768)]
     return out
 
 
@@ -219,6 +244,35 @@
             desc.M >= 1 and desc.M == desc.N * desc.H * desc.W and desc.M * desc.in_ld * 4 < lim and desc.M * desc.out_ld * 4 < lim and
             desc.cout_pad * desc.Cin * 4 < lim and
             (not desc.res or (desc.res_mod if desc.res_mod > 0 else desc.M) * desc.res_ld * 4 < lim))
+
+
+def shortcut_fused_eligible(sc, main, mode=0):
+    lim = 0x7fffff00
+    for d in (sc, main):
+        if (d.KH != 1 or d.KW != 1 or d.pad != 0 or d.mask or d.in_lp or d.out_lp or d.w_packed or d.ksplit > 1 or d.w_batch_rows or d.res or
+                d.Cin < 32 or d.Cin % 32 or d.in_ld < d.Cin or d.in_ld % 4 or d.N < 1 or d.H < 1 or d.W < 1 or not d.inp or not d.w):
+            return False
+    return (mode == 0 and bool(main.out) and main.stride == 1 and sc.stride in (1, 2) and main.M >= 1 and main.M == main.N * main.H * main.W and
+            sc.Ho == (sc.H - 1) // sc.stride + 1 and sc.Wo == (sc.W - 1) // sc.stride + 1 and sc.M == sc.N * sc.Ho * sc.Wo and
+            sc.M == main.M and sc.Cout == main.Cout and main.Cout >= 1 and main.out_ld >= main.Cout and
+            min(sc.cout_pad, main.cout_pad) >= (main.Cout + 63) // 64 * 64 and
+            sc.N * sc.H * sc.W * sc.in_ld * 4 < lim and main.M * main.in_ld * 4 < lim and main.M * main.out_ld * 4 < lim and
+            main.cout_pad * main.Cin * 4 < lim and sc.cout_pad * sc.Cin * 4 < lim)
+
+
+def shortcut_fused_cfg_options(sc, main):
+    out = []
+    for tc in range(4):
+        bn = WINO_GEMM_TILES[tc & 3][1]
+        if (bn > 64 and main.Cout < 128) or min(sc.cout_pad, main.cout_pad) < (main.Cout + bn - 1) // bn * bn:
+            continue
+        out += [(tc, w) for w in (256, 512, 768)]
+    return out
+
+
+def shortcut_fused_launch(sc, main, tile_cfg, wgs):
+    check(_lib.lib().vfn_conv1x1_shortcut_fused_f32(C.byref(sc), C.byref(main), int(tile_cfg), int(wgs), stream()),
+          'vfn_conv1x1_shortcut_fused_f32')
 
 
 def pconv_cfg_options(cout):
@@ -240,6 +294,13 @@
         return
     if cfg >= WINO_GEMM_CFG0:
         c, rows = cfg - WINO_GEMM_CFG0, desc.w_batch_rows
+        if is_wino_gemm32_cfg(cfg):
+            c = cfg - WINO_GEMM32_CFG0
+            if mode != 0 or rows <= 0:
+                raise RuntimeError('the 32-row tiles take an f32 Winograd-domain descriptor (w_batch_rows)')
+            check(_lib.lib().vfn_winograd_gemm_f32(desc.inp, desc.w, desc.out, desc.M // rows, rows, desc.Cin, desc.Cout, desc.cout_pad,
+                                                   8 + (c & 7), (c >> 3) * 128, stream()), 'vfn_winograd_gemm_f32')
+            return
         if mode == 1 and rows > 0:
             check(_lib.lib().vfn_winograd_gemm_bf16(desc.inp, desc.w, desc.out, desc.M // rows, rows, desc.Cin, desc.Cout, desc.cout_pad, c & 7,
                                                     (c >> 3) * 128, stream()), 'vfn_winograd_gemm_bf16')
@@ -256,9 +317,8 @@
 def conv_cfg_name(cfg, mode=0, _cache={}):
     cfg = int(cfg)
     if cfg >= WINO_GEMM_CFG0:
-        c = (cfg - (PCONV_CFG0 if cfg >= PCONV_CFG0 else WINO_GEMM_CFG0)) & 7
-        bm, bn, wm, wn = WINO_GEMM_TILES[c & 3]
-        return f'wino_gemm_kernel<{bm}, {bn}, {wm}, {wn}, {1 + (c >> 2)}, {"true" if cfg >= PCONV_CFG0 else "false"}, {"true" if mode == 1 else "false"}>'
+        bm, bn, wm, wn, pd, _ = persistent_cfg_info(cfg)
+        return f'wino_gemm_kernel<{bm}, {bn}, {wm}, {wn}, {pd}, {"true" if cfg >= PCONV_CFG0 else "false"}, {"true" if mode == 1 else "false"}>'
     if mode not in _cache:
         _cache[mode] = conv_cfg_names(mode)
     return _cache[mode][cfg]
```

New measurement: 167.9, median of 6. 1.01x the previous value.
